# cmaestre/pcl_tracking

Hardware: AMD Instinct MI355X
Metric: particles x input-points / sec per frame (tracked frames/sec @8192 particles per GPU) (higher is better)
Workload: dtype f32

## Files before the change

include/pft.h:

```cpp
#ifndef PFT_H
#define PFT_H

#include <stddef.h>
#include <stdint.h>

#ifdef __cplusplus
extern "C" {
#endif

#define PFT_ABI_VERSION 5

typedef struct pft_point_xyzrgba {
  float x, y, z, w;
  uint32_t rgba;
  uint32_t pad[3];
} pft_point_xyzrgba;

typedef struct pft_particle {
  float x, y, z, w;
  float roll, pitch, yaw, weight;
} pft_particle;

typedef enum pft_status {
  PFT_OK = 0,
// ... 143 lines not shown
  int32_t min_pairs;
  double pair_distance;
  double inlier_distance;
  double margin;
  double trans_eps, rot_eps;
  int32_t apply;
} pft_refine_config;

typedef struct pft_refine_score {
  uint32_t n_pairs, n_inliers;
  double sum_sq_dist, inlier_sq_dist;
} pft_refine_score;

typedef struct pft_refine_result {
  uint32_t status, iterations, n_reference, n_crop;
  double bbox[6];
  float start[12], transform[12];
  pft_particle pose;
  pft_refine_score before, after;
  uint32_t improved, applied;
} pft_refine_result;

typedef struct pft_refine_trace_entry {
  float transform[12];
  uint32_t n_pairs, n_inliers;
  double sums[PFT_REFINE_N_SUMS];
  double step_t2, step_r2;
} pft_refine_trace_entry;

void pft_refine_config_default(pft_refine_config* cfg);
int pft_refine(pft_tracker* t, const float* start12, const pft_refine_config* cfg, pft_refine_result* out);
int pft_get_refine_trace(pft_tracker* t, pft_refine_trace_entry* entries, size_t cap, size_t* n);

typedef struct pft_population_stats {
  double   sum_w, sum_w2;
  double   s[6];
  double   S[21];
  double   n_eff;
  double   mean[6];
  double   cov[36];
  double   rpy_sigma[3];
  float    pos_sigma[3];
  float    pos_axes[9];
  float    w_max;
  uint32_t n, n_zero, i_max, solve_info;
  uint32_t evaluated, uncertain, streak, flagged, calls;
} pft_population_stats;

int pft_set_spread_threshold(pft_tracker* t, double max_pos_sigma, double min_n_eff, int after);
int pft_get_spread_threshold(pft_tracker* t, double* max_pos_sigma, double* min_n_eff, int* after);
int pft_spread(pft_tracker* t);
int pft_get_spread(pft_tracker* t, pft_population_stats* out);

int pft_dist_bind(pft_tracker* t, void* bbox6_dev, void* shard_dev, void* gathered_dev);
int pft_dist_begin_frame(pft_tracker* t);
int pft_dist_phase_a(pft_tracker* t, int iteration);
int pft_dist_phase_b(pft_tracker* t);
int pft_dist_phase_c(pft_tracker* t);

int pft_set_particles(pft_tracker* t, const pft_particle* p, size_t n);
int pft_eval_weights(pft_tracker* t, const pft_particle* particles, size_t P, float* raw_w, int32_t* nn_idx,
                     float* nn_d2);
int pft_debug_get_bbox(pft_tracker* t, float bbox[6]);
int pft_debug_get_crop(pft_tracker* t, int32_t* idx, size_t cap, size_t* n);
int pft_debug_get_input_records(pft_tracker* t, void* out, size_t first, size_t n);
int pft_debug_get_octree(pft_tracker* t, int32_t* depth, double min_xyz[3], double max_xyz[3], uint32_t* n_leaves,
                         uint32_t* n_nodes);
int pft_debug_get_point_keys(pft_tracker* t, uint32_t* keys3, size_t cap_points);
int pft_debug_get_scan_stats(pft_tracker* t, uint64_t* queries, uint64_t* scanned_points);
#define PFT_TREE_INFO_WORDS 64
int pft_debug_get_tree(pft_tracker* t, uint32_t* info, uint32_t* words, size_t words_cap, uint32_t* leaf_order,
                       size_t leaf_order_cap, void* leaf_pts, size_t leaf_pts_cap, void* crop_pts, size_t crop_pts_cap,
                       uint16_t* jump, size_t jump_cap);
int pft_debug_set_limits(pft_tracker* t, uint32_t max_words, int sorted_npass);
int pft_debug_state_save(pft_tracker* t);
int pft_debug_state_restore(pft_tracker* t);
int pft_debug_inject_error(pft_tracker* t, uint32_t bits);
int pft_debug_get_host_stat(pft_tracker* t, uint32_t out4[4]);
int pft_debug_get_ticks(pft_tracker* t, uint64_t* ticks32);
int pft_debug_get_descent_stats(pft_tracker* t, uint64_t* dbg32);
int pft_debug_get_hard_steps(pft_tracker* t, uint64_t out5[5]);
int pft_debug_get_likelihood_layout(pft_tracker* t, uint32_t out4[4]);
int pft_debug_get_ancestor_table(pft_tracker* t, uint32_t info10[10], uint32_t* table, size_t cap);
int pft_debug_aabb_support_subset(const pft_point_xyzrgba* pts, size_t n, uint32_t* keep, size_t* n_keep);
#ifdef PFT_DIAG
void pft_debug_set_ablate(pft_tracker* t, int mask);
#endif
int pft_debug_likelihood_occupancy(void);
int pft_debug_normalize(pft_tracker* t, float* w_inout, size_t n, double* fit_ratio);
int pft_debug_alias(pft_tracker* t, const float* w, size_t n, int32_t* a, double* q);
int pft_debug_weighted_mean(pft_tracker* t, const pft_particle* p, size_t n, pft_particle* out);
int pft_debug_init_particles(pft_tracker* t, const pft_particle* rep, uint32_t id_offset, size_t n_local,
                             pft_particle* out);
int pft_debug_resample(pft_tracker* t, const pft_particle* old, size_t n_total, const int32_t* a, const double* q,
                       const pft_particle* rep, uint32_t epoch, uint32_t id_offset, size_t n_local,
                       pft_particle* out);
int pft_debug_resample_prefix(pft_tracker* t, const pft_particle* old, size_t n_total, const pft_particle* rep,
                              uint32_t epoch, uint32_t id_offset, size_t n_local, int instance, pft_particle* out,
                              float* mats12);
int pft_debug_pose_to_matrix(pft_tracker* t, const pft_particle* p, size_t n, float* m12);
int pft_debug_kld_resample(pft_tracker* t, const pft_particle* old, size_t n_old, const int32_t* a, const double* q,
                           const pft_particle* motion, uint32_t epoch, pft_particle* out, int32_t* bins6,
                           uint32_t* n_out, uint32_t* k_out);
double pft_kld_normal_quantile(double u);
double pft_kld_bound(int k, double delta, double epsilon);

enum {
  PFT_K_RESAMPLE = 0, PFT_K_AABB = 1, PFT_K_CROP = 2, PFT_K_OCTREE = 3, PFT_K_LIKELIHOOD = 4,
  PFT_K_POPULATION = 5, PFT_K_PACK = 6, PFT_K_COUNT = 7
};
int pft_profile_enable(pft_tracker* t, int on);
int pft_profile_get(pft_tracker* t, int kernel_id, double* total_ms, uint64_t* launches);
int pft_profile_reset(pft_tracker* t);
const char* pft_kernel_name(int kernel_id);

#ifdef __cplusplus
}
#endif
#endif
```

pcl_tracking_amd/_lib.py:

```python
import ctypes as C
import os

_HERE = os.path.dirname(os.path.abspath(__file__))
LIB_PATH = os.environ.get("PFT_LIB_PATH") or os.path.join(_HERE, "_build", "libpft_hip.so")

PFT_ABI_VERSION = 5
PFT_SUM_TREE, PFT_SUM_PCL = 0, 1
PFT_CD_RING = 32
PFT_TREE_INFO_WORDS = 64
K_RESAMPLE, K_AABB, K_CROP, K_OCTREE, K_LIKELIHOOD, K_POPULATION, K_PACK, K_COUNT = range(8)

STATUS = {0: "ok", 1: "invalid argument", 2: "no input cloud", 3: "no reference cloud", 4: "no usable HIP device",
          5: "HIP error", 6: "capacity exceeded", 7: "invalid state", 8: "object not recognized"}


class PftError(RuntimeError):
    def __init__(self, status, detail=""):
        self.status = status
        super().__init__("pft status %d (%s) %s" % (status, STATUS.get(status, "?"), detail))


class Config(C.Structure):
    _fields_ = [
        ("abi_version", C.c_uint32), ("device_id", C.c_int32), ("stream", C.c_void_p),
# ... 97 lines not shown
        ("abi_version", C.c_uint32), ("device_id", C.c_int32), ("stream", C.c_void_p),
        ("stream_is_external", C.c_int32),
        ("pass_enable", C.c_int32), ("pass_field", C.c_int32), ("pass_min", C.c_float), ("pass_max", C.c_float),
        ("pass_negative", C.c_int32),
        ("voxel_mode", C.c_int32), ("leaf_size", C.c_float * 3), ("approx_hist_size", C.c_uint32),
        ("max_points", C.c_uint32),
    ]


VOXEL_NONE, VOXEL_APPROX, VOXEL_EXACT = 0, 1, 2


class SegmentConfig(C.Structure):
    _fields_ = [
        ("abi_version", C.c_uint32), ("device_id", C.c_int32), ("stream", C.c_void_p),
        ("stream_is_external", C.c_int32),
        ("transform_enable", C.c_int32), ("transform", C.c_float * 16),
        ("plane_enable", C.c_int32), ("max_iterations", C.c_int32), ("distance_threshold", C.c_double),
        ("probability", C.c_double), ("seed", C.c_uint32), ("optimize_coefficients", C.c_int32),
        ("box_enable", C.c_int32 * 3), ("box_min", C.c_float * 3), ("box_max", C.c_float * 3),
        ("cluster_tolerance", C.c_double), ("min_cluster_size", C.c_int32), ("max_cluster_size", C.c_int32),
        ("max_points", C.c_uint32),
    ]


class SegmentPlane(C.Structure):
    _fields_ = [
        ("status", C.c_int32), ("n_valid", C.c_uint32), ("coefficients", C.c_float * 4),
        ("ransac_coefficients", C.c_float * 4), ("sample", C.c_int32 * 3), ("ransac_inliers", C.c_uint32),
        ("inliers", C.c_uint32), ("iterations", C.c_uint32), ("hypotheses_scored", C.c_uint32),
        ("n_survivors", C.c_uint32),
    ]


PLANE_FOUND, PLANE_NONE, PLANE_DISABLED = 0, 1, 2
SEGMENT_MAX_PLANES = 16
ROUNDS_STOP_FRACTION, ROUNDS_STOP_NO_PLANE, ROUNDS_STOP_MAX_PLANES = 0, 1, 2
SEGMENT_STAGES = ("compaction", "sample", "score", "replay", "refit", "cluster", "output")
MODEL_STAGES = ("remove_zero_points", "centroid", "recentre", "grid_sample")

_vp, _sz, _i32, _u32, _u64, _f64 = C.c_void_p, C.c_size_t, C.c_int32, C.c_uint32, C.c_uint64, C.c_double
_P = C.POINTER
SYMBOLS = [
    ("pft_config_default", None, [_P(Config)]),
    ("pft_status_string", C.c_char_p, [C.c_int]),
    ("pft_create", C.c_int, [_P(Config), _P(_vp)]),
    ("pft_destroy", None, [_vp]),
    ("pft_last_error_string", C.c_char_p, [_vp]),
    ("pft_set_reference", C.c_int, [_vp, _vp, _sz]),
    ("pft_set_trans", C.c_int, [_vp, _vp]),
    ("pft_set_input", C.c_int, [_vp, _vp, _sz]),
    ("pft_set_input_device", C.c_int, [_vp, _vp, _sz]),
    ("pft_set_input_from_filter", C.c_int, [_vp, _vp, _sz]),
    ("pft_compute", C.c_int, [_vp]),
    ("pft_get_result", C.c_int, [_vp, _vp]),
    ("pft_get_particles", C.c_int, [_vp, _vp, _sz, _P(_sz)]),
    ("pft_to_matrix", None, [_vp, _vp]),
    ("pft_to_state", None, [_vp, _vp]),
    ("pft_get_fit_ratio", C.c_int, [_vp, _P(_f64)]),
    ("pft_synchronize", C.c_int, [_vp]),
    ("pft_dist_bind", C.c_int, [_vp, _vp, _vp, _vp]),
    ("pft_dist_begin_frame", C.c_int, [_vp]),
    ("pft_dist_phase_a", C.c_int, [_vp, C.c_int]),
    ("pft_dist_phase_b", C.c_int, [_vp]),
    ("pft_dist_phase_c", C.c_int, [_vp]),
    ("pft_set_particles", C.c_int, [_vp, _vp, _sz]),
    ("pft_eval_weights", C.c_int, [_vp, _vp, _sz, _vp, _vp, _vp]),
    ("pft_debug_get_bbox", C.c_int, [_vp, _vp]),
    ("pft_debug_get_crop", C.c_int, [_vp, _vp, _sz, _P(_sz)]),
    ("pft_debug_get_input_records", C.c_int, [_vp, _vp, _sz, _sz]),
    ("pft_debug_get_octree", C.c_int, [_vp, _P(_i32), _vp, _vp, _P(_u32), _P(_u32)]),
    ("pft_debug_get_point_keys", C.c_int, [_vp, _vp, _sz]),
    ("pft_debug_get_tree", C.c_int, [_vp, _vp, _vp, _sz, _vp, _sz, _vp, _sz, _vp, _sz, _vp, _sz]),
    ("pft_debug_get_scan_stats", C.c_int, [_vp, _P(_u64), _P(_u64)]),
    ("pft_debug_set_limits", C.c_int, [_vp, _u32, C.c_int]),
    ("pft_debug_inject_error", C.c_int, [_vp, _u32]),
    ("pft_debug_state_save", C.c_int, [_vp]),
    ("pft_debug_state_restore", C.c_int, [_vp]),
    ("pft_debug_get_host_stat", C.c_int, [_vp, _vp]),
    ("pft_debug_get_ticks", C.c_int, [_vp, _vp]),
    ("pft_debug_get_descent_stats", C.c_int, [_vp, _vp]),
    ("pft_debug_get_likelihood_layout", C.c_int, [_vp, _vp]),
    ("pft_debug_get_ancestor_table", C.c_int, [_vp, _vp, _vp, _sz]),
    ("pft_debug_get_hard_steps", C.c_int, [_vp, _vp]),
    ("pft_debug_aabb_support_subset", C.c_int, [_vp, C.c_size_t, _vp, _vp]),
    ("pft_debug_likelihood_occupancy", C.c_int, []),
    ("pft_debug_normalize", C.c_int, [_vp, _vp, _sz, _P(_f64)]),
    ("pft_debug_alias", C.c_int, [_vp, _vp, _sz, _vp, _vp]),
    ("pft_debug_weighted_mean", C.c_int, [_vp, _vp, _sz, _vp]),
    ("pft_debug_init_particles", C.c_int, [_vp, _vp, _u32, _sz, _vp]),
    ("pft_debug_resample", C.c_int, [_vp, _vp, _sz, _vp, _vp, _vp, _u32, _u32, _sz, _vp]),
    ("pft_debug_resample_prefix", C.c_int, [_vp, _vp, _sz, _vp, _u32, _u32, _sz, C.c_int, _vp, _vp]),
    ("pft_debug_pose_to_matrix", C.c_int, [_vp, _vp, _sz, _vp]),
    ("pft_debug_kld_resample", C.c_int, [_vp, _vp, _sz, _vp, _vp, _vp, _u32, _vp, _vp, _P(_u32), _P(_u32)]),
    ("pft_set_change_detector", C.c_int, [_vp, C.c_int, C.c_int, C.c_int, _f64]),
    ("pft_get_change_detector", C.c_int, [_vp, _P(C.c_int), _P(C.c_int), _P(C.c_int), _P(_f64)]),
    ("pft_debug_change_state", C.c_int, [_vp, C.c_int, _P(_u32), _P(_u32), _vp, _P(_i32), _vp, _P(_u32)]),
    ("pft_debug_change_detect", C.c_int, [_vp, _vp, _sz, C.c_int, _f64, C.c_int, _vp, _sz, _P(_sz)]),
    ("pft_set_report_cloud", C.c_int, [_vp, _vp, _sz]),
    ("pft_report", C.c_int, [_vp]),
    ("pft_get_report", C.c_int, [_vp, _P(ObjectReport)]),
    ("pft_get_tracked_cloud", C.c_int, [_vp, _vp, _sz, _P(_sz)]),
    ("pft_set_match_threshold", C.c_int, [_vp, _f64, C.c_int]),
    ("pft_get_match_threshold", C.c_int, [_vp, _P(_f64), _P(C.c_int)]),
    ("pft_match", C.c_int, [_vp]),
    ("pft_get_match", C.c_int, [_vp, _P(MatchStatsStruct)]),
    ("pft_get_match_pairs", C.c_int, [_vp, _vp, _vp, _sz, _P(_sz)]),
    ("pft_reset_tracking", C.c_int, [_vp]),
    ("pft_set_spread_threshold", C.c_int, [_vp, _f64, _f64, C.c_int]),
    ("pft_get_spread_threshold", C.c_int, [_vp, _P(_f64), _P(_f64), _P(C.c_int)]),
    ("pft_spread", C.c_int, [_vp]),
    ("pft_get_spread", C.c_int, [_vp, _P(PopulationStatsStruct)]),
    ("pft_reacquire_config_default", None, [_P(ReacquireConfig)]),
    ("pft_reacquire", C.c_int, [_vp, _vp, _sz, _P(ReacquireConfig), _P(ReacquireResultStruct)]),
    ("pft_reacquire_from_segmenter", C.c_int, [_vp, _vp, _P(ReacquireConfig), _P(ReacquireResultStruct)]),
    ("pft_get_reacquire_scores", C.c_int, [_vp, _vp, _vp, _vp, _vp, _vp, _vp, _vp, _vp, _sz, _P(_sz)]),
    ("pft_refine_config_default", None, [_P(RefineConfig)]),
    ("pft_refine", C.c_int, [_vp, _vp, _P(RefineConfig), _P(RefineResultStruct)]),
    ("pft_get_refine_trace", C.c_int, [_vp, _vp, _sz, _P(_sz)]),
    ("pft_kld_normal_quantile", _f64, [_f64]),
    ("pft_kld_bound", _f64, [C.c_int, _f64, _f64]),
    ("pft_profile_enable", C.c_int, [_vp, C.c_int]),
    ("pft_profile_get", C.c_int, [_vp, C.c_int, _P(_f64), _P(_u64)]),
    ("pft_profile_reset", C.c_int, [_vp]),
    ("pft_kernel_name", C.c_char_p, [C.c_int]),
    ("pft_filter_default_config", None, [_P(FilterConfig)]),
    ("pft_filter_create", C.c_int, [_P(FilterConfig), _P(_vp)]),
    ("pft_filter_destroy", None, [_vp]),
    ("pft_filter_last_error_string", C.c_char_p, [_vp]),
    ("pft_filter_apply", C.c_int, [_vp, _vp, _sz]),
    ("pft_filter_apply_device", C.c_int, [_vp, _vp, _sz]),
    ("pft_filter_apply_async", C.c_int, [_vp, _vp, _sz]),
    ("pft_filter_apply_device_async", C.c_int, [_vp, _vp, _sz]),
    ("pft_filter_counts", C.c_int, [_vp, _P(_sz), _P(_sz)]),
    ("pft_filter_output_device", C.c_int, [_vp, _P(_vp), _P(_sz)]),
    ("pft_filter_get_output", C.c_int, [_vp, _vp, _sz, _P(_sz)]),
    ("pft_filter_get_pass_indices", C.c_int, [_vp, _vp, _sz, _P(_sz)]),
    ("pft_filter_last_ms", C.c_int, [_vp, _P(_f64)]),
    ("pft_segment_default_config", None, [_P(SegmentConfig)]),
    ("pft_segment_create", C.c_int, [_P(SegmentConfig), _P(_vp)]),
    ("pft_segment_destroy", None, [_vp]),
    ("pft_segment_last_error_string", C.c_char_p, [_vp]),
    ("pft_segment_apply", C.c_int, [_vp, _vp, _sz]),
    ("pft_segment_apply_device", C.c_int, [_vp, _vp, _sz]),
    ("pft_segment_get_plane", C.c_int, [_vp, _P(SegmentPlane)]),
    ("pft_segment_get_plane_inliers", C.c_int, [_vp, C.c_int, _vp, _sz, _P(_sz)]),
    ("pft_segment_cluster_count", C.c_int, [_vp, _P(_sz)]),
    ("pft_segment_cluster_sizes", C.c_int, [_vp, _vp, _sz]),
    ("pft_segment_get_cluster_indices", C.c_int, [_vp, _vp, _sz, _P(_sz)]),
    ("pft_segment_get_cluster_points", C.c_int, [_vp, _vp, _sz, _P(_sz)]),
    ("pft_segment_last_ms", C.c_int, [_vp, _P(_f64), _vp]),
    ("pft_debug_segment_hypotheses", C.c_int, [_vp, _vp, _vp, _sz, _P(_sz)]),
    ("pft_segment_set_plane_rounds", C.c_int, [_vp, C.c_int, _f64]),
    ("pft_segment_get_plane_rounds", C.c_int, [_vp, _P(C.c_int), _P(_f64)]),
    ("pft_segment_plane_count", C.c_int, [_vp, _P(_sz), _P(C.c_int)]),
    ("pft_segment_get_plane_round", C.c_int, [_vp, _sz, _P(SegmentPlane)]),
    ("pft_segment_get_plane_round_inliers", C.c_int, [_vp, _sz, C.c_int, _vp, _sz, _P(_sz)]),
    ("pft_segment_set_refit_order", C.c_int, [_vp, C.c_int]),
    ("pft_debug_segment_round_hypotheses", C.c_int, [_vp, _sz, _vp, _vp, _sz, _P(_sz)]),
    ("pft_segment_clusters_device", C.c_int, [_vp, _P(_vp), _P(_sz)]),
    ("pft_model_create", C.c_int, [C.c_int, _P(_vp)]),
    ("pft_model_destroy", None, [_vp]),
    ("pft_model_last_error_string", C.c_char_p, [_vp]),
    ("pft_model_prepare", C.c_int, [_vp, _vp, _sz, C.c_float]),
    ("pft_model_prepare_device", C.c_int, [_vp, _vp, _sz, C.c_float]),
    ("pft_model_prepare_from_segment", C.c_int, [_vp, _vp, _sz, C.c_float]),
# ... 58 lines not shown
```

pcl_tracking_amd/csrc/pft_api.hip:

```cpp
#include <math.h>
#include <stdio.h>
#include <string.h>

#include <stdlib.h>

#include <algorithm>
#include <cmath>
#include <string>
#include <vector>

#include "pft_internal.h"
#include "../../include/pft_segment.h"

#define HIPCHK(t, call)                                                                       \
  do {                                                                                        \
    hipError_t e_ = (call);                                                                   \
    if (e_ != hipSuccess) {                                                                   \
      (t)->err = std::string(#call) + ": " + hipGetErrorString(e_);                           \
      return PFT_ERR_HIP;                                                                     \
    }                                                                                         \
  } while (0)

struct EvPair {
  hipEvent_t a, b;
// ... 72 lines not shown
  PftHeader* d_hdr = nullptr;
  int32_t* d_nn_idx = nullptr;
  float* d_nn_d2 = nullptr;
  size_t nn_cap = 0;
  pft_particle* d_dbg_part = nullptr;
  size_t dbg_part_cap = 0;
  PftHeader* d_dbg_hdr = nullptr;
  float* d_dbg_f = nullptr;
  size_t dbg_f_cap = 0;
  void *bound_bbox6 = nullptr, *bound_shard = nullptr, *bound_gathered = nullptr;

  pft_particle* sv_part = nullptr;
  int32_t* sv_alias_list = nullptr;
  double* sv_alias_pref = nullptr;
  uint32_t* sv_alias_pos = nullptr;
  PftHeader* sv_hdr = nullptr;
  int sv_cur = 0;
  uint32_t sv_epoch = 0;
  bool sv_changed = false, sv_valid = false;

  int cd_use = 0;
  uint32_t cd_interval = 10, cd_min_points = 10;
  double cd_res = 0.01, cd_res_latched = 0.01;
  bool cd_latched = false, cd_ever = false, gate_on = false;
  uint32_t cd_counter = 0;
  CdInst cd, cd_dbg;
  double cd_dbg_res = 0.01;
  PftChangeState* sv_cd = nullptr;
  unsigned long long* sv_cd_key[2] = {nullptr, nullptr};
  uint32_t* sv_cd_cnt[2] = {nullptr, nullptr};
  uint32_t sv_cd_cap = 0;
  bool sv_cd_valid = false;
  uint32_t sv_cd_counter = 0;

  pft_point_xyzrgba* d_rep_pts = nullptr;
  pft_point_xyzrgba* d_rep_tracked = nullptr;
  pft_object_report* d_report = nullptr;
  uint32_t rep_n = 0, rep_cap = 0;
  uint32_t rep_tracked_n = 0;
  bool rep_issued = false;

  pft_match_stats* d_match = nullptr;
  int32_t* d_match_idx = nullptr;
  float* d_match_d2 = nullptr;
  uint32_t match_cap = 0;
  uint32_t match_n = 0;
  bool match_issued = false;
  bool tree_of_compute = false;
  double match_min_ratio = 0.0;
  int match_lost_after = 1;

  pft_population_stats* d_spread = nullptr;
  double* d_spread_part = nullptr;
  uint32_t *d_spread_zero = nullptr, *d_spread_imax = nullptr;
  float* d_spread_wmax = nullptr;
  bool spread_issued = false;
  double spread_max_pos_sigma = INFINITY, spread_min_n_eff = 0.0;
  int spread_after = 1;

  pft_particle* d_rq_part = nullptr;
  float* d_rq_mats = nullptr;
  PftRqScores rq_sc = {};
  uint32_t rq_cap = 0;
  float* d_rq_centres = nullptr;
  uint32_t *d_rq_first = nullptr, *d_rq_count = nullptr;
  uint32_t rq_centres_cap = 0;
  float* d_rq_bbox_part = nullptr;
  pft_reacquire_result* d_rq_result = nullptr;
  uint32_t rq_n = 0;
  bool rq_valid = false;
  std::vector<float> rq_centres;
  PftRefineDev rf = {};
  float* d_rf_mats = nullptr;
  uint32_t rf_n = 0;
  bool rf_valid = false;

  bool has_ref = false, has_input = false, initialized = false, changed = false;
  uint32_t resample_epoch = 0;
  float trans[16];

  bool use_graph = false;
  hipGraphExec_t graph_exec = nullptr;
  uint32_t graph_frames = 0, graph_rebuilds = 0;

  bool prof = false;
  std::vector<EvPair> ev[PFT_K_COUNT];
  std::vector<EvPair> ev_free;
  double prof_ms[PFT_K_COUNT] = {0};
  uint64_t prof_n[PFT_K_COUNT] = {0};
};

static const char* k_names[PFT_K_COUNT] = {"resample", "aabb", "crop", "octree", "likelihood", "population", "pack"};

extern "C" const char* pft_kernel_name(int id) { return (id >= 0 && id < PFT_K_COUNT) ? k_names[id] : "?"; }

extern "C" const char* pft_status_string(int s) {
  switch (s) {
    case PFT_OK: return "ok";
    case PFT_ERR_INVALID_ARG: return "invalid argument";
    case PFT_ERR_NO_INPUT: return "no input cloud";
    case PFT_ERR_NO_REFERENCE: return "no reference cloud";
    case PFT_ERR_NO_DEVICE: return "no usable HIP device (there is no CPU fallback)";
    case PFT_ERR_HIP: return "HIP error";
    case PFT_ERR_CAPACITY: return "capacity exceeded";
    case PFT_ERR_STATE: return "invalid state";
    case PFT_ERR_LOST: return "object not recognized";
  }
  return "unknown";
}

extern "C" void pft_config_default(pft_config* c) {
  memset(c, 0, sizeof(*c));
  c->abi_version = PFT_ABI_VERSION;
  c->device_id = 0;
  c->stream = nullptr;
  c->stream_is_external = 0;
  c->particle_num = 400;
  c->iteration_num = 2;
  for (int k = 0; k < 6; k++) {
    c->step_noise_cov[k] = 0.015 * 0.015;
    c->initial_noise_cov[k] = 0.00001;
    c->initial_noise_mean[k] = 0.0;
  }
  c->step_noise_cov[3] *= 40.0;
  c->step_noise_cov[4] *= 40.0;
  c->step_noise_cov[5] *= 40.0;
  c->alpha = 15.0;
  c->resample_likelihood_thr = 0.0;
  c->max_distance = 0.1;
  c->octree_resolution = 0.01;
  c->distance_weight = 1.0;
  c->hsv_weight = 0.1;
  c->h_weight = 1.0;
  c->s_weight = 1.0;
  c->v_weight = 0.0;
  c->hsv_pcl180_argorder = 1;
  c->use_normal = 0;
  c->seed = 1;
  c->rank = 0;
  c->world_size = 1;
  c->kld_adaptive = 0;
  c->maximum_particle_num = 500;
  c->kld_delta = 0.99;
  c->kld_epsilon = 0.2;
  for (int k = 0; k < 6; k++) c->kld_bin_size[k] = 0.1;
  c->motion_ratio = 0.25;
  c->exact_nearest = 0;
  c->sum_order = PFT_SUM_TREE;
}

extern "C" double pft_kld_normal_quantile(double u) {
  static const double a[9] = {1.24818987e-4, -1.075204047e-3, 5.198775019e-3, -0.019198292004, 0.059054035642,
                              -0.151968751364, 0.319152932694, -0.5319230073, 0.797884560593};
  static const double b[15] = {-4.5255659e-5, 1.5252929e-4, -1.9538132e-5, -6.76904986e-4, 1.390604284e-3,
                               -7.9462082e-4, -2.034254874e-3, 6.549791214e-3, -0.010557625006, 0.011630447319,
                               -9.279453341e-3, 5.353579108e-3, -2.141268741e-3, 5.35310849e-4, 9.99936657524e-1};
  double w, y, z;
  if (u == 0.) return 0.5;
  y = u / 2.0;
  if (y < -6.) return 0.0;
  if (y > 6.) return 1.0;
  if (y < 0.) y = -y;
  if (y < 1.) {
    w = y * y;
    z = a[0];
    for (int i = 1; i < 9; i++) z = z * w + a[i];
// ... 221 lines not shown
  dfree(t->sort.keys[0]); dfree(t->sort.keys[1]); dfree(t->sort.vals[0]); dfree(t->sort.vals[1]);
  dfree(t->sort.hist); dfree(t->sort.tile_cnt); dfree(t->sort.tile_box);
  uint32_t cap = n;
  t->max_words = cap * 8u + 64u;
  HIPCHK(t, dalloc(&t->d_in_raw, cap));
  HIPCHK(t, dalloc(&t->d_in_pts, cap));
  HIPCHK(t, dalloc(&t->d_crop_counts, (size_t)(cap / 1024 + 2)));
  HIPCHK(t, dalloc(&t->d_crop_slots, (size_t)(cap / 1024 + 2)));
  HIPCHK(t, hipMemsetAsync(t->d_crop_slots, 0, (size_t)(cap / 1024 + 2) * sizeof(unsigned long long), t->stream));
  HIPCHK(t, dalloc(&t->d_crop_pts, cap));
  HIPCHK(t, dalloc(&t->d_crop_idx, cap));
  HIPCHK(t, dalloc(&t->d_words, t->max_words));
  HIPCHK(t, dalloc(&t->d_leaf_pts, cap));
  HIPCHK(t, dalloc(&t->d_leaf_order, cap));
  HIPCHK(t, dalloc(&t->d_pt_node, cap));
  HIPCHK(t, dalloc(&t->d_pt_key, (size_t)cap * 3));
  HIPCHK(t, dalloc(&t->d_pt_tmp, cap));
  HIPCHK(t, dalloc(&t->d_pt_key64, cap));
  t->sort.ntiles = (cap + 1023u) / 1024u;
  HIPCHK(t, dalloc(&t->sort.keys[0], cap));
  HIPCHK(t, dalloc(&t->sort.keys[1], cap));
  HIPCHK(t, dalloc(&t->sort.vals[0], cap));
  HIPCHK(t, dalloc(&t->sort.vals[1], cap));
  HIPCHK(t, dalloc(&t->sort.hist, (size_t)256 * t->sort.ntiles + 256));
  HIPCHK(t, dalloc(&t->sort.tile_cnt, (size_t)t->sort.ntiles * (PFT_MAX_DEPTH + 2)));
  HIPCHK(t, dalloc(&t->sort.tile_box, (size_t)t->sort.ntiles * 6));
  t->in_cap = cap;
  return PFT_OK;
}

static void cd_free(CdInst& c) {
  dfree(c.b.st); dfree(c.b.set_key[0]); dfree(c.b.set_key[1]); dfree(c.b.set_cnt[0]); dfree(c.b.set_cnt[1]);
  dfree(c.b.tab_key); dfree(c.b.tab_cnt); dfree(c.b.pt_key); dfree(c.b.mark); dfree(c.pts);
  c.b.cap = c.b.tab_cap = 0;
}
static int cd_reserve(pft_tracker* t, CdInst& c, uint32_t cap, bool debug) {
  if (cap < 1024u) cap = 1024u;
  if (c.b.st && cap <= c.b.cap) return PFT_OK;
  CdInst n;
  uint32_t tab = 64u;
  while (tab < 4u * cap) tab <<= 1;
  HIPCHK(t, dalloc(&n.b.st, 1));
  for (int k = 0; k < 2; k++) {
    HIPCHK(t, dalloc(&n.b.set_key[k], cap));
    HIPCHK(t, dalloc(&n.b.set_cnt[k], cap));
  }
  HIPCHK(t, dalloc(&n.b.tab_key, tab));
  HIPCHK(t, dalloc(&n.b.tab_cnt, tab));
  HIPCHK(t, dalloc(&n.b.pt_key, cap));
  if (debug) {
    HIPCHK(t, dalloc(&n.b.mark, cap));
    HIPCHK(t, dalloc(&n.pts, cap));
  }
  n.b.cap = cap;
  n.b.tab_cap = tab;
  if (c.b.st) {
    HIPCHK(t, hipMemcpyAsync(n.b.st, c.b.st, sizeof(PftChangeState), hipMemcpyDeviceToDevice, t->stream));
    for (int k = 0; k < 2; k++) {
      HIPCHK(t, hipMemcpyAsync(n.b.set_key[k], c.b.set_key[k], (size_t)c.b.cap * 8u, hipMemcpyDeviceToDevice, t->stream));
      HIPCHK(t, hipMemcpyAsync(n.b.set_cnt[k], c.b.set_cnt[k], (size_t)c.b.cap * 4u, hipMemcpyDeviceToDevice, t->stream));
    }
    HIPCHK(t, hipStreamSynchronize(t->stream));
  } else {
    HIPCHK(t, hipMemsetAsync(n.b.st, 0, sizeof(PftChangeState), t->stream));
  }
  cd_free(c);
  c = n;
  return PFT_OK;
}

PftSwitches pft_read_switches() {
  auto on = [](const char* name) { return getenv(name) != nullptr; };
  auto is1 = [](const char* name) { const char* e = getenv(name); return e && e[0] == '1'; };
  PftSwitches w = {};
  w.graph = is1("PFT_GRAPH");
  if (const char* b = getenv("PFT_FORCE_BUILDER")) w.builder = !strcmp(b, "single") ? 1 : (!strcmp(b, "sorted") ? 2 : 0);
  w.leaf_indirect = on("PFT_LEAF_INDIRECT") ? (int)is1("PFT_LEAF_INDIRECT") : -1;
  w.aabb_full = on("PFT_AABB_FULL");
  w.resample_one_lane = on("PFT_RESAMPLE_ONE_LANE");
  w.split_resample = on("PFT_SPLIT_RESAMPLE") || w.resample_one_lane;
  w.crop_two_pass = on("PFT_CROP_TWO_PASS");
  w.generic_descent = is1("PFT_GENERIC_DESCENT");
  w.ancestor_table = !on("PFT_ANCESTOR_TABLE") || is1("PFT_ANCESTOR_TABLE");
  w.exact_path = on("PFT_EXACT_SHELLS_ONLY") ? PftExactPath::shells : on("PFT_EXACT_PER_QUERY") ? PftExactPath::per_query : PftExactPath::sorted;
#ifdef PFT_DIAG
  if (const char* a = getenv("PFT_ABLATE")) w.ablate = atoi(a);
  w.skip_octree = on("PFT_DEBUG_SKIP_OCTREE");
#endif
  return w;
}

#ifdef PFT_DIAG
extern "C" void pft_debug_set_ablate(pft_tracker* t, int mask) { if (t) t->sw.ablate = mask; }
#endif

extern "C" int pft_create(const pft_config* cfg, pft_tracker** out) {
  if (!cfg || !out) return PFT_ERR_INVALID_ARG;
  *out = nullptr;
  if (cfg->abi_version != PFT_ABI_VERSION || cfg->particle_num <= 0 || cfg->iteration_num <= 0 ||
      cfg->world_size <= 0 || cfg->rank < 0 || cfg->rank >= cfg->world_size || cfg->use_normal != 0 ||
      cfg->particle_num % cfg->world_size != 0 || !(cfg->octree_resolution > 0) ||
      (cfg->sum_order != PFT_SUM_TREE && cfg->sum_order != PFT_SUM_PCL))
    return PFT_ERR_INVALID_ARG;
  if (cfg->particle_num > PFT_MAX_PARTICLES) return PFT_ERR_CAPACITY;
  if (cfg->kld_adaptive) {
    if (cfg->world_size != 1 || cfg->maximum_particle_num <= 0 || !(cfg->kld_epsilon > 0)) return PFT_ERR_INVALID_ARG;
    for (int k = 0; k < 6; k++)
      if (!(cfg->kld_bin_size[k] > 0)) return PFT_ERR_INVALID_ARG;
    if (cfg->maximum_particle_num >= PFT_POPM_MIN || cfg->particle_num >= PFT_POPM_MIN) return PFT_ERR_CAPACITY;
  }
  int ndev = 0;
  if (hipGetDeviceCount(&ndev) != hipSuccess || ndev <= 0 || cfg->device_id >= ndev) return PFT_ERR_NO_DEVICE;
  if (hipSetDevice(cfg->device_id) != hipSuccess) return PFT_ERR_NO_DEVICE;
  hipDeviceProp_t prop;
  if (hipGetDeviceProperties(&prop, cfg->device_id) != hipSuccess) return PFT_ERR_NO_DEVICE;

  pft_tracker* t = new pft_tracker();
  t->cfg = *cfg;
  t->num_cus = prop.multiProcessorCount > 0 ? prop.multiProcessorCount : 256;
  if (cfg->stream_is_external) {
    t->stream = static_cast<hipStream_t>(cfg->stream);
  } else {
    if (hipStreamCreateWithFlags(&t->stream, hipStreamNonBlocking) != hipSuccess) {
      delete t;
      return PFT_ERR_HIP;
    }
    t->own_stream = true;
  }
  for (int i = 0; i < 16; i++) t->trans[i] = (i % 5 == 0) ? 1.0f : 0.0f;
  t->sw = pft_read_switches();
  t->use_graph = t->sw.graph && t->own_stream;

  PftParams& p = t->prm;
  memset(&p, 0, sizeof(p));
  p.alpha = cfg->alpha;
  p.maxd2 = cfg->max_distance * cfg->max_distance;
  p.res = cfg->octree_resolution;
  p.dist_w = cfg->distance_weight;
  p.hsv_w = cfg->hsv_weight;
  p.h_w = (float)cfg->h_weight;
  p.s_w = (float)cfg->s_weight;
  p.v_w = (float)cfg->v_weight;
  p.hsv_argorder = cfg->hsv_pcl180_argorder;
  for (int k = 0; k < 6; k++) {
    p.step_sigma[k] = sqrt(cfg->step_noise_cov[k]);
    p.init_sigma[k] = sqrt(cfg->initial_noise_cov[k]);
    p.init_mean[k] = cfg->initial_noise_mean[k];
  }
  p.seed_lo = (uint32_t)cfg->seed;
  p.seed_hi = (uint32_t)(cfg->seed >> 32);
  p.P_total = (uint32_t)cfg->particle_num;
  p.P_local = p.P_total / (uint32_t)cfg->world_size;
  p.id_offset = p.P_local * (uint32_t)cfg->rank;
  p.M = 0;
  p.nchunk = 1;
  p.ref_chunk = PFT_REF_CHUNK;
  p.split_last = 0;
  p.kld = cfg->kld_adaptive ? 1u : 0u;
  p.kld_max = (uint32_t)cfg->maximum_particle_num;
  p.kld_z = pft_kld_normal_quantile(cfg->kld_delta);
  p.kld_eps = cfg->kld_epsilon;
  for (int k = 0; k < 6; k++) p.kld_bin[k] = (float)cfg->kld_bin_size[k];
  p.motion_ratio = cfg->motion_ratio;
  p.sum_order = cfg->sum_order;
  t->Pcap = p.kld && p.kld_max > p.P_total ? p.kld_max : p.P_total;

// ... 290 lines not shown
  }
  if (!t->d_n_in) {
    HIPCHK(t, dalloc(&t->d_n_in, 1));
    HIPCHK(t, hipMemsetAsync(t->d_n_in, 0, sizeof(uint32_t), t->stream));
  }
  if (!t->borrow || !t->borrow->filter_alive || t->borrow_of != f) {
    release_borrow(t);
    PftBorrow* b = new PftBorrow();
    if (hipEventCreateWithFlags(&b->ev, hipEventDisableTiming) != hipSuccess) {
      delete b;
      t->err = "pft_set_input_from_filter: hipEventCreateWithFlags failed";
      return PFT_ERR_HIP;
    }
    t->borrow = b;
    t->borrow_of = f;
    pftf_attach(f, b);
  }
  t->borrow->armed = true;
  t->borrow->valid = true;
  HIPCHK(t, hipStreamWaitEvent(t->stream, v.done, 0));
  t->N = (uint32_t)bound;
  t->n_on_device = true;
  t->n_src = v.n_out_dev;
  t->raw_pending = v.out;
  t->has_input = true;
  sync_dev(t);
  return PFT_OK;
}

static void stage_init_particles(pft_tracker* t) {
  pft_particle rep;
  pft_to_state(t->trans, &rep);
  rep.weight = 1.0f / (float)t->prm.P_total;
  sync_dev(t);
  ProfScope ps(t, PFT_K_RESAMPLE);
  pftk_init_particles(t->stream, t->prm, rep, t->d_part[t->cur], t->d_mats, t->d_hdr);
  t->initialized = true;
  t->changed = false;
  t->resample_epoch = 0;
}

static void stage_resample(pft_tracker* t) {
  sync_dev(t);
  pft_particle* out = t->d_part[1 - t->cur];
  {
    ProfScope ps(t, PFT_K_RESAMPLE);
    if (t->prm.kld)
      pftk_resample_kld(t->stream, t->prm, t->dev, t->resample_epoch, out, nullptr, nullptr, nullptr);
    else
      pftk_resample(t->stream, t->prm, t->dev, t->resample_epoch, out, t->sw.resample_one_lane);
  }
  t->resample_epoch++;
  t->cur = 1 - t->cur;
  sync_dev(t);
}

static void stage_aabb(pft_tracker* t, const PftDev& d, uint32_t np, bool finalize) {
  ProfScope ps(t, PFT_K_AABB);
  pftk_aabb(t->stream, t->prm, d, np, finalize);
}
static void stage_resample_aabb(pft_tracker* t, bool finalize) {
  if (!t->prm.kld && t->changed && !t->sw.split_resample) {
    sync_dev(t);
    uint32_t nparts;
    {
      ProfScope ps(t, PFT_K_RESAMPLE);
      nparts = pftk_resample_box(t->stream, t->prm, t->dev, t->resample_epoch, t->d_part[1 - t->cur]);
    }
    if (nparts) {
      t->resample_epoch++;
      t->cur = 1 - t->cur;
      sync_dev(t);
      t->dev.bbox_grid = nparts;
      if (finalize) pftk_bbox_final(t->stream, t->dev);
      return;
    }
  }
  if (t->changed) stage_resample(t);
  sync_dev(t);
  stage_aabb(t, t->dev, t->prm.kld ? t->Pcap : t->prm.P_local, finalize);
}
__global__ void k_inject_error(PftHeader* hdr, uint32_t bits) { hdr->error |= bits; }

static void stage_crop_octree_likelihood(pft_tracker* t, const PftDev& d, uint32_t np, bool debug_nn,
                                         bool bbox_from_partials, bool keep_point_keys = false,
                                         bool likelihood = true) {
  {
    ProfScope ps(t, PFT_K_CROP);
    if (++t->crop_epoch == 0) t->crop_epoch = 1;
    const bool from_filter = t->n_on_device && t->raw_pending;
    pftk_crop(t->stream, t->prm, d, bbox_from_partials, t->crop_epoch, t->raw_pending, t->sw.crop_two_pass,
              from_filter ? t->n_src : nullptr);
    t->raw_pending = nullptr;
    if (from_filter && t->borrow) {
      hipEventRecord(t->borrow->ev, t->stream);
      t->borrow->recorded = true;
      t->borrow->armed = false;
    }
    if (t->inject_error & ~16u) {
      hipLaunchKernelGGL(k_inject_error, dim3(1), dim3(1), 0, t->stream, t->d_hdr, t->inject_error & ~16u);
      t->inject_error &= 16u;
    }
    if (t->gate_on) {
      PftChangeArgs a;
      a.res = t->cd_res_latched;
      a.use = t->cd_use ? 1u : 0u;
      a.interval = t->cd_interval;
      a.min_points = t->cd_min_points;
      a.force = 0u;
      pftk_change_detect(t->stream, t->cd.b, t->d_crop_pts, &t->d_hdr->n_crop, 0u, a, t->h_stat);
    }
  }
  if (t->cfg.exact_nearest) {
    PftDev dq = d;
    {
      const unsigned long long nq = (unsigned long long)np * t->prm.M;
      if (nq > t->eq_cap && nq <= (1ull << 30)) {
        dfree(t->d_eq_sorted); dfree(t->d_eq_out); dfree(t->d_eq_blk); dfree(t->d_eq_tiles);
        t->eq_cap = t->eq_blk_cap = t->eq_tiles_cap = 0;
        const size_t nblk = (size_t)(nq / 64u) + PFT_EC_SLOTS + 64u;
        size_t ppw = ((size_t)np + (size_t)t->num_cus - 1u) / (size_t)t->num_cus;
        ppw = ppw < 1u ? 1u : (ppw > 32u ? 32u : ppw);
        const size_t ntiles = ((size_t)np + ppw - 1u) / ppw + 1u;
        if (dalloc(&t->d_eq_sorted, (size_t)nq) == hipSuccess && dalloc(&t->d_eq_out, (size_t)nq) == hipSuccess &&
            dalloc(&t->d_eq_blk, nblk) == hipSuccess) {
          t->eq_cap = (uint32_t)nq;
          t->eq_blk_cap = (uint32_t)nblk;
          const size_t want = ntiles < 4096u ? ntiles : 4096u;
          if (dalloc(&t->d_eq_tiles, want * 2u * 8192u) == hipSuccess) t->eq_tiles_cap = (uint32_t)want;
          else (void)hipGetLastError();
        } else {
          (void)hipGetLastError();
          dfree(t->d_eq_sorted); dfree(t->d_eq_out); dfree(t->d_eq_blk);
        }
      }
      {
        const volatile uint32_t* hs = t->h_stat;
        const uint32_t demand = hs ? hs[4] : 0u;
        if (demand > t->ec_pool_cap && t->ec_pool_cap < PFT_EC_POOL) {
          unsigned long long want = (unsigned long long)demand + demand / 4u;
          uint32_t cap = t->ec_pool_cap;
          while (cap < want && cap < PFT_EC_POOL) cap <<= 1;
          hipStreamSynchronize(t->stream);
          float4* grown = nullptr;
          if (dalloc(&grown, (size_t)cap) == hipSuccess) {
            dfree(t->d_ec_list);
            t->d_ec_list = grown;
            t->ec_pool_cap = cap;
          } else {
            (void)hipGetLastError();
          }
        }
        dq.ec_list = t->d_ec_list;
        dq.ec_pool_cap = t->ec_pool_cap;
        t->dev.ec_list = t->d_ec_list;
        t->dev.ec_pool_cap = t->ec_pool_cap;
      }
      dq.eq_sorted = t->d_eq_sorted;
      dq.eq_out = t->d_eq_out;
      dq.eq_blk = t->d_eq_blk;
      dq.eq_cap = t->eq_cap;
      dq.eq_blk_cap = t->eq_blk_cap;
      dq.eq_tiles = t->d_eq_tiles;
      dq.eq_tiles_cap = t->eq_tiles_cap;
    }
    {
      ProfScope ps(t, PFT_K_OCTREE);
      pftk_exact_grid(t->stream, t->prm, dq);
    }
    ProfScope ps(t, PFT_K_LIKELIHOOD);
    pftk_likelihood_exact(t->stream, t->prm, dq, np, debug_nn, t->num_cus, t->sw.exact_path);
    return;
  }
  {
    ProfScope ps(t, PFT_K_OCTREE);
    PftDev db = d;
    if (!keep_point_keys) db.pt_key = nullptr;
    const volatile uint32_t* hs = t->h_stat;
    const uint32_t last_n = hs ? hs[0] : 0u, last_depth = hs ? hs[1] : 0u;
    bool sorted = last_n > PFT_SORTED_BUILD_MIN;
    if (t->sw.builder == 1) sorted = false;
    if (t->sw.builder == 2) sorted = true;
#ifdef PFT_DIAG
    if (t->sw.skip_octree && ++t->dbg_builds > 8) {
    } else
#endif
    if (sorted) {
      int npass = last_depth > 0u ? (int)((3u * (last_depth + 1u) + 7u) / 8u) : 8;
      if (t->force_npass > 0) npass = t->force_npass;
      if (npass > 8) npass = 8;
      pftk_octree_sorted(t->stream, t->prm, db, t->sort, d.N, npass);
      t->leaf_indirect = false;
    } else {
      t->leaf_indirect = t->sw.leaf_indirect >= 0 ? t->sw.leaf_indirect == 1 : (unsigned long long)np * t->prm.M <= 8000000ull;
      pftk_octree(t->stream, t->prm, db, last_n, t->leaf_indirect);
    }
  }
  if (!likelihood) return;
  {
    ProfScope ps(t, PFT_K_LIKELIHOOD);
    const int flags = (t->sw.generic_descent ? 0 : 1) | (t->sw.ancestor_table ? 2 : 0) | (t->sw.ablate << 8);
    pftk_likelihood(t->stream, t->prm, d, np, debug_nn, t->num_cus, t->leaf_indirect, flags);
  }
}

static int check_ready(pft_tracker* t) {
  if (!t) return PFT_ERR_INVALID_ARG;
  hipSetDevice(t->cfg.device_id);
  if (!t->has_input || t->N == 0) return PFT_ERR_NO_INPUT;
  if (t->n_on_device && t->raw_pending && !(t->borrow && t->borrow->valid)) {
    t->err = "the filter handed over by pft_set_input_from_filter was applied again or destroyed before the frame's first crop";
    t->has_input = false;
    t->raw_pending = nullptr;
    return PFT_ERR_NO_INPUT;
  }
  if (!t->has_ref) return PFT_ERR_NO_REFERENCE;
  return PFT_OK;
}

extern "C" int pft_compute(pft_tracker* t) {
  int r = check_ready(t);
  if (r != PFT_OK) return r;
  if (t->cfg.world_size != 1) {
    t->err = "pft_compute on a sharded handle: drive the pft_dist_* phases instead";
    return PFT_ERR_STATE;
  }
  t->tree_of_compute = false;
  if (!t->initialized) stage_init_particles(t);
  if (!t->cd_latched) {
    t->cd_res_latched = t->cd_res;
    t->cd_latched = true;
  }
  t->gate_on = t->cd_ever;
  sync_dev(t);
  auto run_iterations = [&]() {
    for (int it = 0; it < t->cfg.iteration_num; it++) {
      stage_resample_aabb(t, false);
      const uint32_t np = t->prm.kld ? t->Pcap : t->prm.P_local;
      stage_crop_octree_likelihood(t, t->dev, np, false, true);
      if (t->inject_error & 16u) {
        hipLaunchKernelGGL(k_inject_error, dim3(1), dim3(1), 0, t->stream, t->d_hdr, 16u);
        t->inject_error &= ~16u;
      }
      {
        ProfScope ps(t, PFT_K_POPULATION);
        pftk_population(t->stream, t->prm, t->dev, t->prm.kld ? t->Pcap : t->prm.P_total, 1, 1, 1, 1);
      }
      t->changed = true;
      if (!t->cd_ever) t->cd_counter = t->cd_counter == 0u ? t->cd_interval : t->cd_counter - 1u;
    }
  };
  const bool graphed = t->use_graph && !t->cfg.exact_nearest && t->changed && !t->prof && !t->n_on_device &&
                       t->graph_frames++ >= 2u;
  if (!graphed) {
    run_iterations();
  } else {
    const int cur0 = t->cur;
    const uint32_t epoch0 = t->resample_epoch, crop0 = t->crop_epoch, grid0 = t->dev.bbox_grid;
    const pft_point_xyzrgba* raw0 = t->raw_pending;
    const uint32_t cdc0 = t->cd_counter;
    hipError_t ge = hipStreamBeginCapture(t->stream, hipStreamCaptureModeThreadLocal);
    hipGraph_t g = nullptr;
    if (ge == hipSuccess) {
      run_iterations();
      ge = hipStreamEndCapture(t->stream, &g);
    }
    if (ge == hipSuccess && g) {
      bool ready = false;
      if (t->graph_exec) {
        hipGraphNode_t bad = nullptr;
        hipGraphExecUpdateResult res;
        ready = hipGraphExecUpdate(t->graph_exec, g, &bad, &res) == hipSuccess;
        if (!ready) {
          (void)hipGetLastError();
          hipGraphExecDestroy(t->graph_exec);
          t->graph_exec = nullptr;
        }
      }
      if (!ready) {
        ge = hipGraphInstantiate(&t->graph_exec, g, nullptr, nullptr, 0);
        t->graph_rebuilds++;
        ready = ge == hipSuccess;
      }
      if (ready) ge = hipGraphLaunch(t->graph_exec, t->stream);
    } else if (ge == hipSuccess) {
      ge = hipErrorUnknown;
    }
    if (g) hipGraphDestroy(g);
    if (ge != hipSuccess) {
      (void)hipGetLastError();
      if (t->graph_exec) {
        hipGraphExecDestroy(t->graph_exec);
        t->graph_exec = nullptr;
      }
      t->use_graph = false;
      t->cur = cur0;
      t->resample_epoch = epoch0;
      t->crop_epoch = crop0;
      t->dev.bbox_grid = grid0;
      t->raw_pending = raw0;
      t->cd_counter = cdc0;
      sync_dev(t);
      run_iterations();
    }
  }
  t->gate_on = false;
  sync_dev(t);
  hipError_t e = hipGetLastError();
  if (e != hipSuccess) {
    t->err = std::string("kernel launch: ") + hipGetErrorString(e);
    return PFT_ERR_HIP;
  }
  t->tree_of_compute = true;
  return PFT_OK;
}

extern "C" int pft_dist_bind(pft_tracker* t, void* bbox6_dev, void* shard_dev, void* gathered_dev) {
  if (!t || !bbox6_dev || !shard_dev || !gathered_dev) return PFT_ERR_INVALID_ARG;
  t->bound_bbox6 = bbox6_dev;
  t->bound_shard = shard_dev;
  t->bound_gathered = gathered_dev;
  sync_dev(t);
  return PFT_OK;
}

extern "C" int pft_dist_begin_frame(pft_tracker* t) {
  int r = check_ready(t);
  if (r != PFT_OK) return r;
  if (!t->bound_gathered) {
    t->err = "pft_dist_bind not called";
    return PFT_ERR_STATE;
  }
  if (!t->initialized) stage_init_particles(t);
  return PFT_OK;
}

extern "C" int pft_dist_phase_a(pft_tracker* t, int iteration) {
  (void)iteration;
  int r = check_ready(t);
  if (r != PFT_OK) return r;
  if (!t->initialized) return PFT_ERR_STATE;
  stage_resample_aabb(t, true);
  return PFT_OK;
}

extern "C" int pft_dist_phase_b(pft_tracker* t) {
  int r = check_ready(t);
  if (r != PFT_OK) return r;
  sync_dev(t);
  stage_crop_octree_likelihood(t, t->dev, t->prm.P_local, false, false);
  {
// ... 170 lines not shown
  t->resample_epoch = t->sv_epoch;
  t->changed = t->sv_changed;
  t->cd_counter = t->sv_cd_counter;
  sync_dev(t);
  CopySegs cs;
  state_segments(t, false, &cs);
  hipLaunchKernelGGL(k_copy_segments, dim3(64, 5), dim3(256), 0, t->stream, cs);
  if (t->sv_cd_valid) {
    const uint32_t cap = t->sv_cd_cap;
    HIPCHK(t, hipMemcpyAsync(t->cd.b.st, t->sv_cd, sizeof(PftChangeState), hipMemcpyDeviceToDevice, t->stream));
    for (int k = 0; k < 2; k++) {
      HIPCHK(t, hipMemcpyAsync(t->cd.b.set_key[k], t->sv_cd_key[k], (size_t)cap * 8u, hipMemcpyDeviceToDevice, t->stream));
      HIPCHK(t, hipMemcpyAsync(t->cd.b.set_cnt[k], t->sv_cd_cnt[k], (size_t)cap * 4u, hipMemcpyDeviceToDevice, t->stream));
    }
  }
  return PFT_OK;
}

extern "C" int pft_debug_inject_error(pft_tracker* t, uint32_t bits) {
  if (!t) return PFT_ERR_INVALID_ARG;
  t->inject_error = bits;
  return PFT_OK;
}
extern "C" int pft_debug_get_host_stat(pft_tracker* t, uint32_t out4[4]) {
  if (!t || !out4 || !t->h_stat) return PFT_ERR_INVALID_ARG;
  for (int i = 0; i < 4; i++) out4[i] = ((volatile uint32_t*)t->h_stat)[i];
  return PFT_OK;
}
static int ensure_dbg_part(pft_tracker* t, size_t n) {
  if (n > t->dbg_part_cap) {
    hipStreamSynchronize(t->stream);
    dfree(t->d_dbg_part);
    HIPCHK(t, dalloc(&t->d_dbg_part, n));
    t->dbg_part_cap = n;
  }
  return PFT_OK;
}
static int ensure_dbg_f(pft_tracker* t, size_t n) {
  if (n > t->dbg_f_cap) {
    hipStreamSynchronize(t->stream);
    dfree(t->d_dbg_f);
    HIPCHK(t, dalloc(&t->d_dbg_f, n));
    t->dbg_f_cap = n;
  }
  return PFT_OK;
}

extern "C" int pft_eval_weights(pft_tracker* t, const pft_particle* particles, size_t P, float* raw_w,
                                int32_t* nn_idx, float* nn_d2) {
  int r = check_ready(t);
  if (r != PFT_OK) return r;
  if (!particles || !P) return PFT_ERR_INVALID_ARG;
  if (P > (t->prm.kld ? t->Pcap : t->prm.P_local)) {
    t->err = "pft_eval_weights: " + std::to_string(P) + " particles handed over, the handle's buffers hold " +
             std::to_string(t->prm.kld ? t->Pcap : t->prm.P_local) + " (particle_num / maximum_particle_num of this rank)";
    return PFT_ERR_CAPACITY;
  }
  r = ensure_dbg_part(t, P);
  if (r != PFT_OK) return r;
  r = ensure_dbg_f(t, P);
  if (r != PFT_OK) return r;
  const bool want_nn = nn_idx || nn_d2;
  const size_t pairs = P * (size_t)t->prm.M;
  if (want_nn && pairs > t->nn_cap) {
    hipStreamSynchronize(t->stream);
    dfree(t->d_nn_idx);
    dfree(t->d_nn_d2);
    HIPCHK(t, dalloc(&t->d_nn_idx, pairs));
    HIPCHK(t, dalloc(&t->d_nn_d2, pairs));
    t->nn_cap = pairs;
  }
  sync_dev(t);
  t->tree_of_compute = false;
  PftDev d = t->dev;
  d.p_active = nullptr;
  d.part_cur = t->d_dbg_part;
  d.part_all = t->d_dbg_part;
  d.bbox6 = t->d_bbox6;
  HIPCHK(t, hipMemcpyAsync(t->d_dbg_part, particles, P * sizeof(pft_particle), hipMemcpyHostToDevice, t->stream));
  HIPCHK(t, hipMemsetAsync(&t->d_hdr->stat_queries, 0, (2 + 32) * sizeof(unsigned long long), t->stream));
  HIPCHK(t, hipMemsetAsync(t->d_hdr->dbg_hard, 0, sizeof(t->d_hdr->dbg_hard) + sizeof(t->d_hdr->lik_layout), t->stream));
  pftk_pose_to_matrix(t->stream, t->d_dbg_part, (uint32_t)P, t->d_mats);
  stage_aabb(t, d, (uint32_t)P, false);
  stage_crop_octree_likelihood(t, d, (uint32_t)P, want_nn, true, true);
  pftk_finalize_raw(t->stream, t->prm, d, (uint32_t)P, t->d_dbg_f, nullptr);
  if (raw_w) HIPCHK(t, hipMemcpyAsync(raw_w, t->d_dbg_f, P * sizeof(float), hipMemcpyDeviceToHost, t->stream));
  if (nn_idx) HIPCHK(t, hipMemcpyAsync(nn_idx, t->d_nn_idx, pairs * sizeof(int32_t), hipMemcpyDeviceToHost, t->stream));
  if (nn_d2) HIPCHK(t, hipMemcpyAsync(nn_d2, t->d_nn_d2, pairs * sizeof(float), hipMemcpyDeviceToHost, t->stream));
  HIPCHK(t, hipStreamSynchronize(t->stream));
  if (t->initialized) pftk_pose_to_matrix(t->stream, t->d_part[t->cur], t->prm.P_local, t->d_mats);
  HIPCHK(t, hipGetLastError());
  return check_device_error(t);
}

static int read_hdr(pft_tracker* t, PftHeader* h) {
  HIPCHK(t, hipMemcpyAsync(h, t->d_hdr, sizeof(PftHeader), hipMemcpyDeviceToHost, t->stream));
  HIPCHK(t, hipStreamSynchronize(t->stream));
  return PFT_OK;
}

extern "C" int pft_debug_get_bbox(pft_tracker* t, float bbox[6]) {
  if (!t || !bbox) return PFT_ERR_INVALID_ARG;
  PftHeader h;
  int r = read_hdr(t, &h);
  if (r != PFT_OK) return r;
  memcpy(bbox, h.bbox, sizeof(float) * 6);
  return PFT_OK;
}

extern "C" int pft_debug_get_crop(pft_tracker* t, int32_t* idx, size_t cap, size_t* n) {
  if (!t) return PFT_ERR_INVALID_ARG;
  PftHeader h;
  int r = read_hdr(t, &h);
  if (r != PFT_OK) return r;
  if (n) *n = h.n_crop;
  size_t c = cap < h.n_crop ? cap : h.n_crop;
  if (idx && c) {
    HIPCHK(t, hipMemcpy(idx, t->d_crop_idx, c * sizeof(int32_t), hipMemcpyDeviceToHost));
  }
  return PFT_OK;
}

extern "C" int pft_debug_get_input_records(pft_tracker* t, void* out, size_t first, size_t n) {
  if (!t || (!out && n)) return PFT_ERR_INVALID_ARG;
  if (first + n > t->in_cap) return PFT_ERR_CAPACITY;
  hipSetDevice(t->cfg.device_id);
  HIPCHK(t, hipStreamSynchronize(t->stream));
  if (n) HIPCHK(t, hipMemcpy(out, t->d_in_pts + first, n * sizeof(float4), hipMemcpyDeviceToHost));
  return PFT_OK;
}

extern "C" int pft_debug_get_octree(pft_tracker* t, int32_t* depth, double mn[3], double mx[3], uint32_t* n_leaves,
                                    uint32_t* n_nodes) {
  if (!t) return PFT_ERR_INVALID_ARG;
  PftHeader h;
  int r = read_hdr(t, &h);
  if (r != PFT_OK) return r;
  if (h.error) {
    t->err = "octree build error flag " + std::to_string(h.error);
    return PFT_ERR_CAPACITY;
  }
  if (depth) *depth = h.depth;
  if (mn) memcpy(mn, h.omin, sizeof(double) * 3);
  if (mx) memcpy(mx, h.omax, sizeof(double) * 3);
  if (n_leaves) *n_leaves = h.n_leaves;
  if (n_nodes) *n_nodes = h.n_words;
  return PFT_OK;
}

extern "C" int pft_debug_get_point_keys(pft_tracker* t, uint32_t* keys3, size_t cap_points) {
  if (!t || !keys3) return PFT_ERR_INVALID_ARG;
  PftHeader h;
  int r = read_hdr(t, &h);
  if (r != PFT_OK) return r;
  size_t c = cap_points < h.n_crop ? cap_points : h.n_crop;
  if (c) HIPCHK(t, hipMemcpy(keys3, t->d_pt_key, c * 3 * sizeof(uint32_t), hipMemcpyDeviceToHost));
  return PFT_OK;
}

extern "C" int pft_debug_get_tree(pft_tracker* t, uint32_t* info, uint32_t* words, size_t words_cap, uint32_t* leaf_order,
                                  size_t leaf_order_cap, void* leaf_pts, size_t leaf_pts_cap, void* crop_pts,
                                  size_t crop_pts_cap, uint16_t* jump, size_t jump_cap) {
  if (!t || !info) return PFT_ERR_INVALID_ARG;
  if (t->cfg.world_size != 1 || t->cfg.exact_nearest) {
    t->err = "pft_debug_get_tree: sharded handles (world_size > 1) and the exact nearest-neighbour mode build no octree";
    return PFT_ERR_INVALID_ARG;
  }
  if (t->in_cap == 0 || !t->d_words) {
    t->err = "pft_debug_get_tree before the first input cloud: no tree buffers yet";
    return PFT_ERR_STATE;
  }
  hipSetDevice(t->cfg.device_id);
  PftHeader h;
  int r = read_hdr(t, &h);
  if (r != PFT_OK) return r;
  const size_t n_jump = (size_t)1 << (3 * PFT_JUMP_MAX_LEVEL);
  uint32_t f32[5];
  memcpy(&f32[0], &h.margin_cells, 4);
  memcpy(&f32[1], &h.inv_res, 4);
  memcpy(&f32[2], h.ominf, 12);
  memset(info, 0, PFT_TREE_INFO_WORDS * sizeof(uint32_t));
  info[0] = h.n_crop; info[1] = h.error; info[2] = (uint32_t)h.depth; info[3] = (uint32_t)h.use_table;
  info[4] = h.n_words; info[5] = h.n_leaves; info[6] = h.leaf_start; info[7] = (uint32_t)h.n_grow;
  info[8] = (uint32_t)h.build_path; info[9] = (uint32_t)h.leaf_indirect; info[10] = (uint32_t)h.jump_level;
  for (int k = 0; k < 5; k++) info[11 + k] = f32[k];
  info[16] = h.build_epoch; info[17] = h.build_variant;
  info[18] = ((uint32_t)pftk_max_lds_bytes() - 10240u) & ~15u;
  info[19] = (uint32_t)n_jump;
  static_assert(20 + PFT_MAX_DEPTH + 3 <= PFT_TREE_INFO_WORDS, "lvl_start does not fit the info block");
  for (int l = 0; l <= h.depth + 1 && l < PFT_MAX_DEPTH + 3 && h.depth > 0; l++) info[20 + l] = h.lvl_start[l];
  const size_t n_pts = std::min<size_t>(h.n_crop, t->in_cap);
  const size_t n_words = std::min<size_t>(h.n_words, (size_t)t->in_cap * 8u + 64u);
  auto copy = [&](void* dst, const void* src, size_t cap, size_t count, size_t elem) -> hipError_t {
    const size_t c = std::min(cap, count);
    return dst && src && c ? hipMemcpy(dst, src, c * elem, hipMemcpyDeviceToHost) : hipSuccess;
  };
  HIPCHK(t, copy(words, t->d_words, words_cap, n_words, sizeof(uint32_t)));
  HIPCHK(t, copy(leaf_order, t->d_leaf_order, leaf_order_cap, n_pts, sizeof(uint32_t)));
  HIPCHK(t, copy(leaf_pts, t->d_leaf_pts, leaf_pts_cap, n_pts, sizeof(float4)));
  HIPCHK(t, copy(crop_pts, t->d_crop_pts, crop_pts_cap, n_pts, sizeof(float4)));
  HIPCHK(t, copy(jump, t->d_jump, jump_cap, n_jump, sizeof(uint16_t)));
  return PFT_OK;
}

extern "C" int pft_debug_get_ticks(pft_tracker* t, uint64_t* ticks32) {
  if (!t || !ticks32) return PFT_ERR_INVALID_ARG;
  PftHeader h;
  int r = read_hdr(t, &h);
  if (r != PFT_OK) return r;
  for (int i = 0; i < 32; i++) ticks32[i] = h.ticks[i];
  return PFT_OK;
}

extern "C" int pft_debug_aabb_support_subset(const pft_point_xyzrgba* pts, size_t n, uint32_t* keep, size_t* n_keep) {
  if ((!pts && n) || !keep || !n_keep) return PFT_ERR_INVALID_ARG;
  std::vector<uint32_t> k;
  pft_aabb_support_subset(pts, n, k);
  for (size_t i = 0; i < k.size(); i++) keep[i] = k[i];
  *n_keep = k.size();
  return PFT_OK;
}

extern "C" int pft_debug_get_descent_stats(pft_tracker* t, uint64_t* dbg32) {
  if (!t || !dbg32) return PFT_ERR_INVALID_ARG;
  PftHeader h;
  int r = read_hdr(t, &h);
  if (r != PFT_OK) return r;
  for (int i = 0; i < 32; i++) dbg32[i] = h.dbg[i];
  dbg32[30] = t->prm.M_box;
  dbg32[31] = t->prm.M;
  if (t->cfg.exact_nearest) {
    dbg32[8] = h.ec_nslots;
    dbg32[9] = h.ec_pool_used;
    dbg32[10] = h.eq_totals & 0xffffffffull;
    dbg32[11] = h.eq_totals >> 32;
    dbg32[12] = h.eg_ncells;
    dbg32[13] = h.n_crop;
  }
  return PFT_OK;
}

extern "C" int pft_debug_get_likelihood_layout(pft_tracker* t, uint32_t out4[4]) {
  if (!t || !out4) return PFT_ERR_INVALID_ARG;
  PftHeader h;
  int r = read_hdr(t, &h);
  if (r != PFT_OK) return r;
  memcpy(out4, h.lik_layout, sizeof(h.lik_layout));
  return PFT_OK;
}

extern "C" int pft_debug_get_ancestor_table(pft_tracker* t, uint32_t info10[10], uint32_t* table, size_t cap) {
  if (!t || !info10) return PFT_ERR_INVALID_ARG;
  PftHeader h;
  int r = read_hdr(t, &h);
  if (r != PFT_OK) return r;
  const bool has = t->d_anc != nullptr && h.anc_level > 0;
  info10[0] = has && h.anc_epoch == h.build_epoch ? 1u : 0u;
  info10[1] = has ? (uint32_t)h.anc_level : 0u;
  for (int a = 0; a < 3; a++) {
    info10[2 + a] = has ? h.anc_lo[a] : 0u;
    info10[5 + a] = has ? h.anc_bits[a] : 0u;
  }
  info10[8] = h.build_epoch;
  info10[9] = h.anc_epoch;
  const size_t cells = has ? (size_t)1 << (h.anc_bits[0] + h.anc_bits[1] + h.anc_bits[2]) : 0u;
  if (table && cells && cap) {
    HIPCHK(t, hipMemcpyAsync(table, t->d_anc, std::min(cap, cells) * sizeof(uint32_t), hipMemcpyDeviceToHost, t->stream));
    HIPCHK(t, hipStreamSynchronize(t->stream));
  }
  return PFT_OK;
}

extern "C" int pft_debug_get_hard_steps(pft_tracker* t, uint64_t out5[5]) {
  if (!t || !out5) return PFT_ERR_INVALID_ARG;
  PftHeader h;
  int r = read_hdr(t, &h);
  if (r != PFT_OK) return r;
  for (int i = 0; i < 5; i++) out5[i] = h.dbg_hard[i];
  return PFT_OK;
}

extern "C" int pft_debug_get_scan_stats(pft_tracker* t, uint64_t* queries, uint64_t* scanned) {
  if (!t) return PFT_ERR_INVALID_ARG;
  PftHeader h;
  int r = read_hdr(t, &h);
  if (r != PFT_OK) return r;
  if (queries) *queries = h.stat_queries;
  if (scanned) *scanned = h.stat_scanned;
  return PFT_OK;
}

struct DbgPop {
  pft_particle* part = nullptr;
  int32_t* a = nullptr;
  double* q = nullptr;
  int32_t* list = nullptr;
  double* pref = nullptr;
  uint32_t* pos = nullptr;
  ~DbgPop() {
    dfree(part); dfree(a); dfree(q); dfree(list); dfree(pref); dfree(pos);
  }
};

static int dbg_population(pft_tracker* t, std::vector<pft_particle>& host, int norm, int mean, int alias, DbgPop& b,
                          PftHeader* hout) {
  const size_t n = host.size();
  if (n > PFT_MAX_PARTICLES) return PFT_ERR_CAPACITY;
  HIPCHK(t, dalloc(&b.part, n));
  HIPCHK(t, dalloc(&b.a, n));
  HIPCHK(t, dalloc(&b.q, n));
  HIPCHK(t, dalloc(&b.list, 2 * n));
  HIPCHK(t, dalloc(&b.pref, 2 * n));
  HIPCHK(t, dalloc(&b.pos, n));
  HIPCHK(t, hipMemcpyAsync(b.part, host.data(), n * sizeof(pft_particle), hipMemcpyHostToDevice, t->stream));
  HIPCHK(t, hipMemsetAsync(t->d_dbg_hdr, 0, sizeof(PftHeader), t->stream));
  sync_dev(t);
  PftDev d = t->dev;
  d.p_active = nullptr;
  d.part_all = b.part;
  d.alias_list = b.list;
  d.alias_pref = b.pref;
  d.alias_pos = b.pos;
  d.hdr = t->d_dbg_hdr;
  pftk_population(t->stream, t->prm, d, (uint32_t)n, 0, norm, mean, alias);
  if (alias) pftk_alias_materialize(t->stream, d, (uint32_t)n, b.a, b.q);
  HIPCHK(t, hipMemcpyAsync(host.data(), b.part, n * sizeof(pft_particle), hipMemcpyDeviceToHost, t->stream));
  if (hout) HIPCHK(t, hipMemcpyAsync(hout, t->d_dbg_hdr, sizeof(PftHeader), hipMemcpyDeviceToHost, t->stream));
  HIPCHK(t, hipStreamSynchronize(t->stream));
  HIPCHK(t, hipGetLastError());
  return PFT_OK;
// ... 983 lines not shown
```

pcl_tracking_amd/csrc/pft_device_utils.h:

```cpp
#pragma once
#include <float.h>
#include <math.h>

#include "pft_internal.h"

#define WAVE 64
#define UNROLL_FENCE(j, every) do { if (((j) % (every)) == (every) - 1) __builtin_amdgcn_sched_barrier(0); } while (0)

__device__ __forceinline__ bool pft_unchanged(const uint32_t* gate) { return gate && *gate == 0u; }

__device__ __forceinline__ int lane_id() { return threadIdx.x & (WAVE - 1); }
__device__ __forceinline__ int wave_id() { return threadIdx.x >> 6; }

template <typename T>
__device__ __forceinline__ T wave_sum(T v) {
#pragma unroll
  for (int o = 32; o > 0; o >>= 1) v += __shfl_xor(v, o);
  return v;
}
template <int CTRL, int ROW_MASK>
__device__ __forceinline__ double dpp_move_f64(double v) {
  const unsigned long long b = (unsigned long long)__double_as_longlong(v);
  const int lo = __builtin_amdgcn_update_dpp(0, (int)(uint32_t)b, CTRL, ROW_MASK, 0xf, false);
  const int hi = __builtin_amdgcn_update_dpp(0, (int)(uint32_t)(b >> 32), CTRL, ROW_MASK, 0xf, false);
// ... 110 lines not shown
      k1 += 0xBB67AE85u;
    }
    uint32_t hi0 = __umulhi(0xD2511F53u, c0), lo0 = 0xD2511F53u * c0;
    uint32_t hi1 = __umulhi(0xCD9E8D57u, c2), lo1 = 0xCD9E8D57u * c2;
    uint32_t n0 = hi1 ^ c1 ^ k0, n1 = lo1, n2 = hi0 ^ c3 ^ k1, n3 = lo0;
    c0 = n0; c1 = n1; c2 = n2; c3 = n3;
  }
  o[0] = c0; o[1] = c1; o[2] = c2; o[3] = c3;
}

__device__ __forceinline__ double u53(uint32_t a, uint32_t b) {
  unsigned long long m = ((unsigned long long)(a >> 5) << 26) | (unsigned long long)(b >> 6);
  return (double)m * (1.0 / 9007199254740992.0);
}

__device__ __forceinline__ void normal_pair(const PftParams& p, uint32_t pid, uint32_t slot, uint32_t epoch,
                                            uint32_t purpose, double& z0, double& z1) {
  uint32_t o[4];
  philox4x32(pid, slot, epoch, purpose, p.seed_lo, p.seed_hi, o);
  double u1 = 1.0 - u53(o[0], o[1]);
  double u2 = u53(o[2], o[3]);
  double r = sqrt(-2.0 * log(u1));
  double th = 6.283185307179586 * u2;
  z0 = r * cos(th);
  z1 = r * sin(th);
}

__device__ __forceinline__ void particle_sample(pft_particle& q, const PftParams& p, const double* sigma,
                                                const double* mean, uint32_t pid, uint32_t epoch, uint32_t purpose) {
  double z[6];
  normal_pair(p, pid, 1, epoch, purpose, z[0], z[1]);
  normal_pair(p, pid, 2, epoch, purpose, z[2], z[3]);
  normal_pair(p, pid, 3, epoch, purpose, z[4], z[5]);
  q.x += (float)(z[0] * sigma[0] + mean[0]);
  q.y += (float)(z[1] * sigma[1] + mean[1]);
  q.z += (float)(z[2] * sigma[2] + mean[2]);
  q.roll += (float)(z[3] * sigma[3] + mean[3]);
  q.pitch += (float)(z[4] * sigma[4] + mean[4]);
  q.yaw += (float)(z[5] * sigma[5] + mean[5]);
}

__device__ __forceinline__ float sqrt_rn_coherence(float x) {
  float s = __builtin_amdgcn_sqrtf(x);
  const float sd = __uint_as_float(__float_as_uint(s) - 1u), su = __uint_as_float(__float_as_uint(s) + 1u);
  const float ed = fmaf(-sd, s, x), eu = fmaf(-su, s, x);
  s = ed <= 0.0f ? sd : s;
  s = eu > 0.0f ? su : s;
  return s;
}

__device__ __forceinline__ void pose_to_matrix(const pft_particle& q, float* m ) {
  float A = (float)cos((double)q.yaw), B = (float)sin((double)q.yaw);
  float C = (float)cos((double)q.pitch), D = (float)sin((double)q.pitch);
  float E = (float)cos((double)q.roll), F = (float)sin((double)q.roll);
  float DE = D * E, DF = D * F;
  m[0] = A * C;  m[1] = A * DF - B * E;  m[2] = B * F + A * DE;  m[3] = q.x;
  m[4] = B * C;  m[5] = A * E + B * DF;  m[6] = B * DE - A * F;  m[7] = q.y;
  m[8] = -D;     m[9] = C * F;           m[10] = C * E;          m[11] = q.z;
}

__device__ __forceinline__ void store_matrix(float* mats, uint32_t i, const float* m) {
  float4* dst = reinterpret_cast<float4*>(mats + 12 * (size_t)i);
  dst[0] = make_float4(m[0], m[1], m[2], m[3]);
  dst[1] = make_float4(m[4], m[5], m[6], m[7]);
  dst[2] = make_float4(m[8], m[9], m[10], m[11]);
}

__device__ __forceinline__ void load_matrix(const float* mats, uint32_t i, float* T) {
  const float4* tp = reinterpret_cast<const float4*>(mats + 12 * (size_t)i);
  float4 r0 = tp[0], r1 = tp[1], r2 = tp[2];
  T[0] = r0.x; T[1] = r0.y; T[2] = r0.z; T[3] = r0.w;
  T[4] = r1.x; T[5] = r1.y; T[6] = r1.z; T[7] = r1.w;
  T[8] = r2.x; T[9] = r2.y; T[10] = r2.z; T[11] = r2.w;
}

__device__ __forceinline__ void xform(const float* T, float x, float y, float z, float& ox, float& oy, float& oz) {
  ox = T[0] * x + T[1] * y + T[2] * z + T[3];
  oy = T[4] * x + T[5] * y + T[6] * z + T[7];
  oz = T[8] * x + T[9] * y + T[10] * z + T[11];
}

#include "pft_alias.h"

__device__ inline void pft_anc_window(PftHeader* hdr, const PftDev& d, int D, bool on, const double mn[3], double res) {
  const int L = D - PFT_ANC_UP;
  on = on && d.anc != nullptr && L >= 1;
  const float inv = (float)(1.0 / res);
  uint32_t lo[3] = {0u, 0u, 0u}, bits[3] = {0u, 0u, 0u};
  for (int a = 0; a < 3 && on; a++) {
    const float om = (float)mn[a];
    const float f0 = fmaxf(floorf((hdr->bbox[2 * a] - om) * inv), 0.0f);
    const float f1 = fmaxf(floorf((hdr->bbox[2 * a + 1] - om) * inv), 0.0f);
    const uint32_t top = (1u << L) - 1u;
    const uint32_t c0 = min(f0 < 2147483648.0f ? (uint32_t)f0 >> PFT_ANC_UP : top, top);
    const uint32_t c1 = min(f1 < 2147483648.0f ? (uint32_t)f1 >> PFT_ANC_UP : top, top);
    on = c1 >= c0;
    const uint32_t n = c1 - c0 + 1u;
    bits[a] = n > 1u ? 32u - (uint32_t)__clz((int)(n - 1u)) : 0u;
    lo[a] = min(c0, (1u << L) - (1u << bits[a]));
  }
  on = on && bits[0] + bits[1] + bits[2] <= PFT_ANC_CAP_BITS;
  hdr->anc_level = on ? L : 0;
  for (int a = 0; a < 3; a++) {
    hdr->anc_lo[a] = on ? lo[a] : 0u;
    hdr->anc_bits[a] = on ? bits[a] : 0u;
  }
  hdr->build_epoch = hdr->build_epoch + 1u;
}
```

pcl_tracking_amd/csrc/pft_internal.h:

```cpp
#pragma once
#include <hip/hip_runtime.h>
#include <stdint.h>

#include <vector>

#include "../../include/pft.h"

#define PFT_MAX_DEVICES 64
#define PFT_MAX_DEPTH 30
#define PFT_TABLE_MAX_DEPTH 10
#define PFT_MAX_GROW 40
#define PFT_JUMP_MAX_LEVEL 4
#ifndef PFT_ANC_CAP_BITS
#define PFT_ANC_CAP_BITS 18
#endif
#define PFT_ANC_CAP (1u << PFT_ANC_CAP_BITS)
#ifndef PFT_ANC_UP
#define PFT_ANC_UP 2
#endif
#define PFT_REF_CHUNK 256
#ifndef PFT_BUILD_THREADS
#define PFT_BUILD_THREADS 1024
#endif
#ifndef PFT_LIK_GROUPS
#define PFT_LIK_GROUPS 64
#endif
#ifndef PFT_LIK_CTR_STRIDE
#define PFT_LIK_CTR_STRIDE 16u
#endif
#ifndef PFT_LIK_THREADS
#define PFT_LIK_THREADS 1024
#endif
#ifndef PFT_LIK_WGS_PER_CU
#define PFT_LIK_WGS_PER_CU 2
#endif
#define PFT_POP_THREADS 1024
#define PFT_SORTED_BUILD_MIN 18000
#define PFT_EG_CAP (1u << 21)
#define PFT_EC_SLOTS (1u << 19)
#define PFT_EC_POOL (1u << 24)
#define PFT_EC_POOL_MIN (1u << 20)
#define PFT_POPM_THREADS 256
#define PFT_POPM_ITEMS 16
#define PFT_POPM_MAX_WGS 256
#define PFT_POPM_MIN (16 * PFT_POP_THREADS + 1)
#define PFT_MAX_PARTICLES (PFT_POPM_MAX_WGS * PFT_POPM_THREADS * PFT_POPM_ITEMS)

struct PftParams {
  double alpha;
  double maxd2;
  double res;
  double dist_w, hsv_w;
  float h_w, s_w, v_w;
  int hsv_argorder;
  double step_sigma[6], init_sigma[6], init_mean[6];
  uint32_t seed_lo, seed_hi;
  uint32_t P_total, P_local, id_offset;
  uint32_t M, nchunk;
  uint32_t M_box;
  uint32_t ref_chunk;
  uint32_t split_last;
  uint32_t kld;
  uint32_t kld_max;
  double kld_z;
  double kld_eps;
  float kld_bin[6];
  double motion_ratio;
  int32_t sum_order;
};

struct PftHeader {
  float bbox[6];
  uint32_t n_crop;
  uint32_t error;
  double omin[3], omax[3];
  int32_t depth;
  int32_t use_table;
  uint32_t n_words;
  uint32_t n_leaves;
  uint32_t leaf_start;
  uint32_t lvl_start[PFT_MAX_DEPTH + 3];
  int32_t n_grow;
  int32_t build_path;
  uint32_t build_variant;
  int32_t leaf_indirect;
  int32_t jump_level;
  float margin_cells;
  float ominf[3];
  float inv_res;
  int32_t anc_level;
  uint32_t anc_lo[3], anc_bits[3];
  uint32_t build_epoch;
  uint32_t anc_epoch;
  uint32_t grow_idx[PFT_MAX_GROW];
  uint32_t grow_shift[PFT_MAX_GROW];
  uint32_t grow_old_depth[PFT_MAX_GROW];
  double grow_min[PFT_MAX_GROW + 1][3];
  double fit_ratio;
  pft_particle rep;
  pft_particle motion;
  uint32_t alias_m, alias_nh;
  float eg_g, eg_inv_g, eg_min[3];
  int32_t eg_dim[3];
  uint32_t eg_ncells;
  uint32_t p_active;
  uint32_t kld_k;
  unsigned long long stat_queries, stat_scanned;
  unsigned long long dbg[32];
  unsigned long long ticks[32];
  alignas(128) uint32_t lik_ctr[PFT_LIK_GROUPS * PFT_LIK_CTR_STRIDE];
  alignas(128) uint32_t ec_nslots;
  uint32_t ec_pool_used;
  unsigned long long eq_totals;
  alignas(128) uint32_t crop_ticket;
  uint32_t pop_bar[4];
  unsigned long long dbg_hard[5];
  uint32_t lik_layout[4];
};

// ... 57 lines not shown
  uint32_t eq_tiles_cap;
  uint32_t* kld_table;
  int32_t* kld_bins;
  uint32_t* host_stat;
  int32_t* nn_idx;
  float* nn_d2;
  const uint32_t* gate;
};

struct PftChangeState {
  double mn[3], mx[3];
  int32_t depth;
  uint32_t defined;
  uint32_t counter;
  uint32_t gate;
  uint32_t n_set[2];
  uint32_t prev;
  uint32_t n_calls;
  uint32_t ring[PFT_CD_RING][5];
};
struct PftChangeBufs {
  PftChangeState* st;
  unsigned long long* set_key[2];
  uint32_t* set_cnt[2];
  unsigned long long* tab_key;
  uint32_t* tab_cnt;
  unsigned long long* pt_key;
  uint32_t* mark;
  uint32_t cap, tab_cap;
};
struct PftChangeArgs {
  double res;
  uint32_t use, interval, min_points;
  uint32_t force;
};
void pftk_change_detect(hipStream_t s, const PftChangeBufs& b, const float4* pts, const uint32_t* n_ptr, uint32_t n,
                        const PftChangeArgs& a, uint32_t* host_stat);

struct PftBorrow {
  hipEvent_t ev = nullptr;
  bool recorded = false;
  bool armed = false;
  bool valid = false;
  bool tracker_alive = true, filter_alive = true;
};
struct pft_filter;
struct PftFilterView {
  const pft_point_xyzrgba* out;
  const uint32_t* n_out_dev;
  size_t n_in;
  int device_id;
  hipEvent_t done;
};
int pftf_view(pft_filter* f, PftFilterView* v);
void pftf_attach(pft_filter* f, PftBorrow* b);

void pftk_remove_zero_points(hipStream_t s, const pft_point_xyzrgba* in, uint32_t n, float4* xyz, uint8_t* flag,
                             uint32_t* tile, uint32_t* keep_idx, float4* keep_xyz, uint32_t* n_keep);
struct pft_segment;
int pftsg_device_id(const pft_segment* s);
struct pft_model;
struct PftModelView {
  const pft_point_xyzrgba* recentred;
  size_t n_recentred;
  const pft_point_xyzrgba* reference;
  size_t n_reference;
  float trans[16];
  uint32_t first_nonfinite;
  int device_id;
};
int pftm_view(const pft_model* m, PftModelView* v);

enum class PftExactPath { sorted, per_query, shells };
struct PftSwitches {
  bool graph;
  int builder;
  int leaf_indirect;
  bool aabb_full;
  bool split_resample;
  bool resample_one_lane;
  bool crop_two_pass;
  bool generic_descent;
  bool ancestor_table;
  PftExactPath exact_path;
  int ablate;
  bool skip_octree;
};
PftSwitches pft_read_switches();

void pftk_report(hipStream_t s, const pft_point_xyzrgba* pts, uint32_t n, const PftHeader* hdr, int sum_order,
                 pft_point_xyzrgba* tracked, pft_object_report* out);
void pftk_match(hipStream_t s, const PftParams& p, const PftDev& d, double min_ratio, uint32_t lost_after,
                pft_match_stats* out, int32_t* input_idx, float* sq_dist);
uint32_t pftk_spread_blocks(uint32_t n_max);
void pftk_spread(hipStream_t s, const PftDev& d, uint32_t n_max, double* part, uint32_t* part_zero, float* part_wmax,
                 uint32_t* part_imax, double max_pos_sigma, double min_n_eff, uint32_t after, pft_population_stats* out);
struct PftRqLattice {
  uint32_t n[3];
  float base[3], span[3];
};
struct PftRqScores {
  uint32_t *n_inliers, *n_matched;
  double *coherence, *sum_sq_dist, *inlier_sq_dist;
};
void pftk_reacquire_centroids(hipStream_t s, const pft_point_xyzrgba* pts, const uint32_t* first, const uint32_t* count,
                              uint32_t n_clusters, float* centres);
void pftk_reacquire_candidates(hipStream_t s, const float* centres, uint32_t K, const PftRqLattice& lat, pft_particle* part,
                               float* mats);
void pftk_reacquire_score(hipStream_t s, const PftParams& p, const PftDev& d, uint32_t K, double inlier_d2,
                          const PftRqScores& out);
void pftk_reacquire_select(hipStream_t s, const PftParams& p, const PftDev& d, const PftRqScores& sc, uint32_t K,
                           uint32_t n_centres, uint32_t per_centre, double accept_ratio, pft_reacquire_result* out);
struct PftRefineCtl;
struct PftRefineDev {
  PftRefineCtl* ctl;
  double* part;
  uint32_t* part_n;
  uint32_t g_cap;
  pft_refine_result* result;
  pft_refine_trace_entry* trace;
};
struct PftRefineArgs {
  float start[12];
  uint32_t use_rep;
  uint32_t max_iterations, min_pairs;
  double pair2, inl2, margin, trans_eps2, rot_eps2;
};
size_t pftk_refine_ctl_bytes();
uint32_t pftk_refine_blocks(uint32_t M);
void pftk_refine_init(hipStream_t s, const PftRefineArgs& a, const PftRefineDev& r, const PftHeader* hdr, float* mats);
void pftk_refine_passes(hipStream_t s, const PftParams& p, const PftDev& d, const PftRefineDev& r, const PftRefineArgs& a);
void pftk_pack_reference(hipStream_t s, const pft_point_xyzrgba* d_pts, uint32_t n, int argorder, float4* xyz,
                         float4* hsv);
void pftk_pack_input(hipStream_t s, const pft_point_xyzrgba* d_pts, uint32_t n, float4* out,
                     const uint32_t* n_dev = nullptr);
void pftk_init_particles(hipStream_t s, const PftParams& p, pft_particle rep, pft_particle* out, float* mats,
                         PftHeader* hdr);
void pftk_resample(hipStream_t s, const PftParams& p, const PftDev& d, uint32_t epoch, pft_particle* out, bool one_lane);
void pftk_bbox_final(hipStream_t s, const PftDev& d);
uint32_t pftk_resample_box(hipStream_t s, const PftParams& p, const PftDev& d, uint32_t epoch, pft_particle* out);
void pftk_resample_table(hipStream_t s, const PftParams& p, const pft_particle* old, const int32_t* a,
                         const double* q, const PftHeader* hdr, uint32_t epoch, pft_particle* out);
void pftk_pose_to_matrix(hipStream_t s, const pft_particle* p, uint32_t n, float* mats);
void pftk_aabb(hipStream_t s, const PftParams& p, const PftDev& d, uint32_t n_particles, bool finalize);
void pft_aabb_support_subset(const pft_point_xyzrgba* pts, size_t n, std::vector<uint32_t>& keep);
void pftk_exact_grid(hipStream_t s, const PftParams& p, const PftDev& d);
void pftk_likelihood_exact(hipStream_t s, const PftParams& p, const PftDev& d, uint32_t n_particles, bool debug_nn,
                           int num_cus, PftExactPath path);
void pftk_resample_kld(hipStream_t s, const PftParams& p, const PftDev& d, uint32_t epoch, pft_particle* out,
                       const int32_t* table_a, const double* table_q, int32_t* bins_out);
void pftk_crop(hipStream_t s, const PftParams& p, const PftDev& d, bool bbox_from_partials, uint32_t epoch,
               const pft_point_xyzrgba* raw, bool two_pass, const uint32_t* n_src = nullptr);
void pftk_octree(hipStream_t s, const PftParams& p, const PftDev& d, uint32_t expected_points, bool indirect);
void pftk_octree_rescue(hipStream_t s, const PftParams& p, const PftDev& d);
struct SortBufs {
  unsigned long long* keys[2];
  uint32_t* vals[2];
  uint32_t* hist;
  uint32_t* tile_cnt;
  float* tile_box;
  uint32_t ntiles;
};
void pftk_octree_sorted(hipStream_t s, const PftParams& p, const PftDev& d, const SortBufs& sb, uint32_t n_pad,
                        int npass);
void pftk_likelihood(hipStream_t s, const PftParams& p, const PftDev& d, uint32_t n_particles, bool debug_nn,
                     int num_cus, bool leaf_indirect, int flags);
void pftk_finalize_raw(hipStream_t s, const PftParams& p, const PftDev& d, uint32_t n_particles,
                       float* raw_out , pft_particle* shard );
void pftk_population(hipStream_t s, const PftParams& p, const PftDev& d, uint32_t n, int from_partials,
                     int do_normalize, int do_mean, int do_alias);
void pftk_alias_materialize(hipStream_t s, const PftDev& d, uint32_t n, int32_t* a, double* q);
int pftk_max_lds_bytes();
int pftk_cur_device();
int pftk_radix_sort_pairs(hipStream_t s, uint32_t* key[2], uint32_t* val[2], uint32_t n, int bits, uint32_t* hist);
```

pcl_tracking_amd/csrc/pft_likelihood.hip:

```cpp
#include "pft_device_utils.h"

#ifndef PFT_LIK_PENALTY
#define PFT_LIK_PENALTY 1
#endif

struct LikCtx {
  const uint32_t* words;
  const float* tab;
  uint32_t per_axis;
  const float* lut_h;
  const float* lut_s;
  const float* pen;
  const uint16_t* jump;
  int J;
  uint32_t lvlJ_start;
  const uint32_t* anc;
  uint32_t alo, abits;
  float margin, near_thr, ominx, ominy, ominz, inv_res, ncell;
  uint32_t leaf0;
  const uint16_t* leaf16;
};

struct HybridWords {
  const __attribute__((address_space(3))) uint32_t* lds;
  const uint32_t* __restrict__ glob;
  uint32_t n_lds;
  __device__ __forceinline__ uint32_t operator[](uint32_t i) const { return i < n_lds ? lds[i] : glob[i]; }
};

__device__ __forceinline__ double rcp_nr(double x) {
  double r = __builtin_amdgcn_rcp(x);
  double e = fma(-x, r, 1.0);
  r = fma(r, e, r);
  e = fma(-x, r, 1.0);
  r = fma(r, e, r);
  return r;
}

__device__ __forceinline__ bool face_violation(uint32_t kx, uint32_t ky, uint32_t kz, uint32_t lowf, uint32_t highf,
                                               int sh) {
  const uint32_t mx = (1u << sh) - 1u;
  const uint32_t rx = kx & mx, ry = ky & mx, rz = kz & mx;
  bool v = ((lowf & 1u) && rx == 0) || ((highf & 1u) && rx == mx);
  v |= ((lowf & 2u) && ry == 0) || ((highf & 2u) && ry == mx);
  v |= ((lowf & 4u) && rz == 0) || ((highf & 4u) && rz == mx);
  return v;
}

__device__ __forceinline__ int near_face_level(uint32_t k, bool low, bool high) {
  const uint32_t t = low ? k : ~k;
  const uint32_t c = min((uint32_t)(t == 0u ? -1 : __builtin_ctz(t)), 31u);
  return (low | high) ? (int)c : -1;
}

template <bool USE_TAB, bool FAST, bool DEBUG_NN, int LEAF, bool INDIRECT, typename WordPtr>
__device__ __forceinline__ void likelihood_items(const PftParams& prm, const PftDev& d, const LikCtx& cx, WordPtr W,
                                                 uint32_t n_particles, int D, uint32_t n_crop,
                                                 const double omin[3], int abl) {
  const int lane = lane_id(), w = wave_id(), nw = blockDim.x >> 6;
  const uint32_t M = prm.M, nchunk = prm.nchunk;
  const uint32_t G = min((uint32_t)PFT_LIK_GROUPS, gridDim.x), grp = blockIdx.x % G;
  const uint32_t gq = gridDim.x / G, gr = gridDim.x % G;
  const uint32_t wgs_in_grp = gq + (grp < gr ? 1u : 0u), waves_in_grp = wgs_in_grp * (uint32_t)nw;
  const uint32_t wgs_before = grp * gq + min(grp, gr);
  const uint32_t pb = (uint32_t)((unsigned long long)n_particles * wgs_before / gridDim.x);
  const uint32_t pe = (uint32_t)((unsigned long long)n_particles * (wgs_before + wgs_in_grp) / gridDim.x);
  const uint32_t np_grp = pe - pb, nbig = prm.split_last ? nchunk - prm.split_last : nchunk, nsmall = nchunk - nbig;
  const uint32_t small_len = prm.split_last ? prm.ref_chunk / prm.split_last : 0u;
  const uint32_t it_begin = 0u, it_end = np_grp * nchunk, big_items = np_grp * nbig;
  const uint32_t lw = (blockIdx.x / G) * (uint32_t)nw + (uint32_t)w;
  uint32_t* ctr = &d.hdr->lik_ctr[grp * PFT_LIK_CTR_STRIDE];
  const double res = prm.res;
  const double maxd2 = prm.maxd2;
  const double wd = prm.dist_w, whsv = prm.hsv_w;
  const float hw = prm.h_w, sw = prm.s_w, vw = prm.v_w;
  for (uint32_t item_v = it_begin + lw; item_v < it_end;) {
    const uint32_t item = (uint32_t)__builtin_amdgcn_readfirstlane((int)item_v);
    uint32_t pi, ch, cstart, clen;
    if (item < big_items) {
      pi = pb + item / nbig;
      ch = item % nbig;
      cstart = ch * prm.ref_chunk;
      clen = prm.ref_chunk;
    } else {
      const uint32_t r = item - big_items;
      pi = pb + r / nsmall;
      ch = nbig + r % nsmall;
      cstart = nbig * prm.ref_chunk + (r % nsmall) * small_len;
      clen = small_len;
    }
    float T[12];
    load_matrix(d.mats, pi, T);
    double val = 0.0;
    unsigned long long st_q = 0, st_s = 0;
    const uint32_t jend = min(M, cstart + clen);
    const uint32_t j0 = cstart + lane;
    float4 rnext = j0 < jend ? d.ref_xyz[j0] : make_float4(0, 0, 0, 0);
    for (uint32_t j = j0; j < jend; j += WAVE) {
      const float4 r = rnext;
      if (j + WAVE < jend) rnext = d.ref_xyz[j + WAVE];
      float qx, qy, qz;
      xform(T, r.x, r.y, r.z, qx, qy, qz);
      if (n_crop == 0) {
        if (DEBUG_NN) {
          const size_t o = (size_t)pi * M + d.ref_perm[j];
          d.nn_idx[o] = -1;
          d.nn_d2[o] = INFINITY;
        }
        continue;
      }
      uint32_t node = 0, jx = 1, jy = 1, jz = 1;
      int lvl = 0;
      int dbg_fast = 0, dbg_gen = 0, dbg_jump = 0, dbg_hard = 0;
      if (FAST) {
        const float tx = (qx - cx.ominx) * cx.inv_res, ty = (qy - cx.ominy) * cx.inv_res,
                    tz = (qz - cx.ominz) * cx.inv_res;
        const float flx = floorf(tx), fly = floorf(ty), flz = floorf(tz);
        const bool inside = (int)(fminf(fminf(tx, ty), tz) >= 0.0f) & (int)(fmaxf(fmaxf(tx, ty), tz) < cx.ncell);
        const float fx = tx - flx, fy = ty - fly, fz = tz - flz;
        const float mg = cx.margin, mh = 1.0f - cx.margin;
        const uint32_t kx = inside ? (uint32_t)flx : 0u, ky = inside ? (uint32_t)fly : 0u,
                       kz = inside ? (uint32_t)flz : 0u;
        int V = -1;
        const float off = fmaxf(fmaxf(fabsf(fx - 0.5f), fabsf(fy - 0.5f)), fabsf(fz - 0.5f));
        if (__builtin_amdgcn_ballot_w64(off > cx.near_thr)) {
          const int vx = near_face_level(kx, fx < mg, fx > mh), vy = near_face_level(ky, fy < mg, fy > mh),
                    vz = near_face_level(kz, fz < mg, fz > mh);
          V = max(vx, max(vy, vz));
        }
        V = inside ? V : 31;
        int lim = min(D, D - 1 - V);
        bool inw = false;
        uint32_t ae = 0u;
        if (!INDIRECT && LEAF == 1 && cx.anc) {
          const uint32_t bx = cx.abits & 0xffu, by = (cx.abits >> 8) & 0xffu, bz = cx.abits >> 16;
          const uint32_t ux = (kx >> PFT_ANC_UP) - (cx.alo & 1023u), uy = (ky >> PFT_ANC_UP) - ((cx.alo >> 10) & 1023u),
                         uz = (kz >> PFT_ANC_UP) - (cx.alo >> 20);
          inw = ((ux >> bx) | (uy >> by) | (uz >> bz)) == 0u;
          ae = cx.anc[inw ? ux | (uy << bx) | (uz << (bx + by)) : 0u];
        }
        const int a = (int)(ae >> 27);
        const bool hit = inw & (a <= lim);
        node = hit ? (ae & 0x7ffffffu) : 0u;
        lvl = hit ? a : 0;
        lim = (hit & (a < D - PFT_ANC_UP)) ? a : lim;
        if (cx.J > 0 && __builtin_amdgcn_ballot_w64(!hit)) {
          const int sh = D - cx.J;
          const uint32_t e = cx.jump[(kx >> sh) | ((ky >> sh) << cx.J) | ((kz >> sh) << (2 * cx.J))];
          const bool take = !hit & (cx.J <= lim) & (e != 0u);
          node = take ? cx.lvlJ_start + e - 1u : node;
          lvl = take ? cx.J : lvl;
          if (DEBUG_NN) dbg_jump = take ? 1 : 0;
        }
        while (lvl < lim) {
          const int sh = D - lvl - 1;
          const uint32_t c = (((kx >> sh) & 1u) << 2) | (((ky >> sh) & 1u) << 1) | ((kz >> sh) & 1u);
          const uint32_t wv = W[node];
          if (!((wv >> c) & 1u)) break;
          node = (wv >> 8) + __popc(wv & 0xffu & ((1u << c) - 1u));
          lvl++;
          dbg_fast++;
        }
        const int up = D - lvl;
        const uint32_t top = 1u << lvl;
        jx = (kx >> up) | top; jy = (ky >> up) | top; jz = (kz >> up) | top;
      }
      if ((abl & 1) && lvl < D) {
        node = cx.leaf0;
        lvl = D;
      }
      for (; lvl < D; lvl++) {
        dbg_gen++;
        const uint32_t wv = W[node];
        const uint32_t mask = wv & 0xffu, base = wv >> 8;
        float cx0, cx1, cy0, cy1, cz0, cz1;
        if (USE_TAB) {
          const float2 tx2 = *reinterpret_cast<const float2*>(cx.tab - 2 + 2u * jx);
          const float2 ty2 = *reinterpret_cast<const float2*>(cx.tab + cx.per_axis - 2 + 2u * jy);
          const float2 tz2 = *reinterpret_cast<const float2*>(cx.tab + 2u * cx.per_axis - 2 + 2u * jz);
          cx0 = tx2.x; cx1 = tx2.y; cy0 = ty2.x; cy1 = ty2.y; cz0 = tz2.x; cz1 = tz2.y;
        } else {
          const double vs = res * (double)(1u << (D - lvl - 1));
          const uint32_t pkx = jx - (1u << lvl), pky = jy - (1u << lvl), pkz = jz - (1u << lvl);
          cx0 = (float)(((double)(2u * pkx) + 0.5) * vs + omin[0]);
          cx1 = (float)(((double)(2u * pkx + 1u) + 0.5) * vs + omin[0]);
          cy0 = (float)(((double)(2u * pky) + 0.5) * vs + omin[1]);
          cy1 = (float)(((double)(2u * pky + 1u) + 0.5) * vs + omin[1]);
          cz0 = (float)(((double)(2u * pkz) + 0.5) * vs + omin[2]);
          cz1 = (float)(((double)(2u * pkz + 1u) + 0.5) * vs + omin[2]);
        }
        float dx0 = cx0 - qx, dx1 = cx1 - qx, dy0 = cy0 - qy, dy1 = cy1 - qy, dz0 = cz0 - qz, dz1 = cz1 - qz;
        float X0 = dx0 * dx0, X1 = dx1 * dx1, Y0 = dy0 * dy0, Y1 = dy1 * dy1, Z0 = dz0 * dz0, Z1 = dz1 * dz1;
        const float yz[4] = {Y0 + Z0, Y0 + Z1, Y1 + Z0, Y1 + Z1};
#if PFT_LIK_PENALTY
        const float4 pa = *reinterpret_cast<const float4*>(cx.pen + 8u * mask);
        const float4 pb = *reinterpret_cast<const float4*>(cx.pen + 8u * mask + 4u);
        const float d0 = (X0 + yz[0]) + pa.x, d1 = (X0 + yz[1]) + pa.y, d2 = (X0 + yz[2]) + pa.z, d3 = (X0 + yz[3]) + pa.w;
        const float d4 = (X1 + yz[0]) + pb.x, d5 = (X1 + yz[1]) + pb.y, d6 = (X1 + yz[2]) + pb.z, d7 = (X1 + yz[3]) + pb.w;
        float m0, m1, m2, best;
        asm("v_min3_f32 %0, %1, %2, %3" : "=v"(m0) : "v"(d0), "v"(d1), "v"(d2));
        asm("v_min3_f32 %0, %1, %2, %3" : "=v"(m1) : "v"(d3), "v"(d4), "v"(d5));
        asm("v_min3_f32 %0, %1, %2, %3" : "=v"(m2) : "v"(d6), "v"(d7), "v"(m0));
        asm("v_min_f32 %0, %1, %2" : "=v"(best) : "v"(m1), "v"(m2));
        uint32_t bc = 7u;
        bc = d6 == best ? 6u : bc;
        bc = d5 == best ? 5u : bc;
        bc = d4 == best ? 4u : bc;
        bc = d3 == best ? 3u : bc;
        bc = d2 == best ? 2u : bc;
        bc = d1 == best ? 1u : bc;
        bc = d0 == best ? 0u : bc;
#else
        float best = INFINITY;
        uint32_t bc = 0;
#pragma unroll
        for (uint32_t c = 0; c < 8; c++) {
          float dc = ((c & 4u) ? X1 : X0) + yz[c & 3u];
          bool ex = (mask >> c) & 1u;
          if (ex && dc < best) {
            best = dc;
            bc = c;
          }
        }
#endif
        if (DEBUG_NN) {
          const uint32_t ideal = ((X1 < X0) ? 4u : 0u) | ((Y1 < Y0) ? 2u : 0u) | ((Z1 < Z0) ? 1u : 0u);
          if (!((mask >> ideal) & 1u)) dbg_hard++;
        }
        node = base + __popc(mask & ((1u << bc) - 1u));
        jx = 2u * jx + ((bc >> 2) & 1u);
        jy = 2u * jy + ((bc >> 1) & 1u);
        jz = 2u * jz + (bc & 1u);
      }
      uint32_t ls, le;
// ... 47 lines not shown
        if (!(bd < INFINITY)) bpos = d.leaf_order[min(bpos, n_crop - 1u)];
      }
      const float4 bt = INDIRECT ? d.crop_pts[bpos] : d.leaf_pts[bpos];
      if (DEBUG_NN) {
        const size_t o = (size_t)pi * M + d.ref_perm[j];
        d.nn_idx[o] = INDIRECT ? (int32_t)bpos : (int32_t)d.leaf_order[bpos];
        d.nn_d2[o] = bd;
        st_q += 1;
        st_s += le - ls;
        {
          const int first = __ffsll((long long)__ballot(1)) - 1;
          const int gb = dbg_gen < 10 ? dbg_gen : 10, hb = dbg_hard < 4 ? dbg_hard : 4;
          for (int g_ = 0; g_ <= 10; g_++) {
            const unsigned long long m_ = __ballot(gb == g_);
            if (m_ && lane == first) atomicAdd(&d.hdr->dbg[g_], (unsigned long long)__popcll(m_));
          }
          for (int h_ = 0; h_ <= 4; h_++) {
            const unsigned long long m_ = __ballot(hb == h_);
            if (m_ && lane == first) atomicAdd(&d.hdr->dbg_hard[h_], (unsigned long long)__popcll(m_));
          }
          const unsigned long long mj_ = __ballot(dbg_jump != 0);
          if (mj_ && lane == first) atomicAdd(&d.hdr->dbg[11], (unsigned long long)__popcll(mj_));
        }
        int mg_ = dbg_gen, mf_ = dbg_fast, ml_ = (int)(le - ls);
        for (int o = 32; o > 0; o >>= 1) {
          mg_ = max(mg_, __shfl_xor(mg_, o));
          mf_ = max(mf_, __shfl_xor(mf_, o));
          ml_ = max(ml_, __shfl_xor(ml_, o));
        }
        if (lane == __ffsll((long long)__ballot(1)) - 1) {
          atomicAdd(&d.hdr->dbg[12], 1ull);
          atomicAdd(&d.hdr->dbg[13], (unsigned long long)mg_);
          atomicAdd(&d.hdr->dbg[14], (unsigned long long)mf_);
          atomicAdd(&d.hdr->dbg[15], (unsigned long long)ml_);
          atomicAdd(&d.hdr->dbg[16 + (mg_ < 10 ? mg_ : 10)], 1ull);
        }
      }
      if (abl & 4) {
        val += (double)bd;
      } else if ((double)bd < maxd2) {
        float ex = qx - bt.x, ey = qy - bt.y, ez = qz - bt.z;
        float n2 = (ex * ex + ey * ey) + ez * ez;
        double dist = (double)sqrt_rn_coherence(n2);
        double A = 1.0 + dist * dist * wd;
        const float4 rh = d.ref_hsv[j];
        const uint32_t pk = __float_as_uint(bt.w);
        const float th = cx.lut_h[pk & 0xffu], ts = cx.lut_s[(pk >> 8) & 0xffu], tv = cx.lut_s[(pk >> 16) & 0xffu];
        const float hd1 = fabsf(rh.x - th);
        float hd2;
        if (rh.x < th)
          hd2 = fabsf(1.0f + rh.x - th);
        else
          hd2 = fabsf(1.0f + th - rh.x);
        float h_diff;
        if (hd1 < hd2)
          h_diff = hw * hd1 * hd1;
        else
          h_diff = hw * hd2 * hd2;
        const float s_diff = sw * (rh.y - ts) * (rh.y - ts);
        const float v_diff = vw * (rh.z - tv) * (rh.z - tv);
        const float diff2 = h_diff + s_diff + v_diff;
        double Bq = 1.0 + whsv * (double)diff2;
        val += rcp_nr(A * Bq);
      }
    }
    val = wave_sum_lane63(val);
    if (lane == 63) d.partial[(size_t)pi * nchunk + ch] = val;
    {
      uint32_t nx = 0;
      if (lane == 0) nx = it_begin + waves_in_grp + atomicAdd(ctr, 1u);
      item_v = (uint32_t)__shfl((int)nx, 0);
    }
    if (DEBUG_NN) {
      st_q = wave_sum(st_q);
      st_s = wave_sum(st_s);
      if (lane == 0 && st_q) {
        atomicAdd(&d.hdr->stat_queries, st_q);
        atomicAdd(&d.hdr->stat_scanned, st_s);
      }
    }
  }
}

#define PFT_LIK_RUN(UT, FA, LF) likelihood_items<UT, FA, DEBUG_NN, LF, INDIRECT>(prm, d, cx, W, n_particles, D, n_crop, omin, abl)

template <bool DEBUG_NN, bool INDIRECT, bool GATED>
__global__ __launch_bounds__(PFT_LIK_THREADS, DEBUG_NN ? 1 : (PFT_LIK_THREADS * PFT_LIK_WGS_PER_CU) / 256) void k_likelihood(PftParams prm, PftDev d, uint32_t n_particles,
                                                                uint32_t lds_bytes, int flags) {
  const int allow_fast = flags & 1;
#ifdef PFT_DIAG
  const int abl = flags >> 8;
#else
  constexpr int abl = 0;
#endif
  extern __shared__ __attribute__((aligned(16))) unsigned char smem[];
  const PftHeader* hdr = d.hdr;
  if (GATED && pft_unchanged(d.gate)) return;
  if (d.p_active) n_particles = *d.p_active;
  const int D = hdr->depth;
  const uint32_t n_crop = (hdr->error || D <= 0 || (hdr->leaf_indirect != 0) != INDIRECT) ? 0u : hdr->n_crop;
  if (hdr->error && blockIdx.x == 0 && threadIdx.x == 0 && d.host_stat) {
    d.host_stat[2] = hdr->error;
    d.host_stat[3] |= hdr->error;
  }
  const uint32_t n_words = hdr->n_words;
  const int use_tab = hdr->use_table;
  const double omin[3] = {hdr->omin[0], hdr->omin[1], hdr->omin[2]};
  const uint32_t per_axis = use_tab ? (2u << D) : 0u;
  const bool fast = allow_fast && use_tab && hdr->margin_cells < 0.5f;
  int J = fast ? hdr->jump_level : 0;

  float* pen = reinterpret_cast<float*>(smem);
  constexpr uint32_t pen_bytes = PFT_LIK_PENALTY ? 256u * 8u * 4u : 0u;
  float* lut_h = reinterpret_cast<float*>(smem + pen_bytes);
  float* lut_s = lut_h + 256;
  float* tab = lut_s + 256;
  uint32_t used = pen_bytes + 2048u + 3u * per_axis * 4u;
  used = (used + 15u) & ~15u;
  const uint32_t leaf_start = hdr->leaf_start, n_leaves = hdr->n_leaves;
  const bool leaf16 = n_crop > 0 && n_crop < 65536u;
  const uint32_t branch_bytes = leaf16 ? leaf_start * 4u : n_words * 4u;
  const uint32_t leaf_bytes = leaf16 ? ((n_leaves + 1u) * 2u + 3u) & ~3u : 0u;
  uint32_t jump_bytes = J > 0 ? (2u << (3 * J)) : 0u;
  const bool fits_with_jump = (size_t)used + jump_bytes + branch_bytes + leaf_bytes <= (size_t)lds_bytes;
  const bool fits_without_jump = (size_t)used + branch_bytes + leaf_bytes <= (size_t)lds_bytes;
  const bool branch_only = use_tab && !fits_with_jump && leaf16 && (size_t)used + jump_bytes + branch_bytes <= (size_t)lds_bytes;
  const bool jump_dropped = !fits_with_jump && fits_without_jump && !branch_only && J > 0;
  if (!fits_with_jump && fits_without_jump && !branch_only) {
    J = 0;
    jump_bytes = 0;
  }
  uint16_t* ljump = reinterpret_cast<uint16_t*>(smem + used);
  used += jump_bytes;
  uint32_t* lwords = reinterpret_cast<uint32_t*>(smem + used);
  uint16_t* lleaf = reinterpret_cast<uint16_t*>(smem + used + branch_bytes);
  const bool words_in_lds = !branch_only && (size_t)used + branch_bytes + leaf_bytes <= (size_t)lds_bytes;
  const uint32_t n_lds_words = (words_in_lds || branch_only) ? 0u : min(n_words, (lds_bytes - used) / 4u);
  if (DEBUG_NN && blockIdx.x == 0 && threadIdx.x == 0) {
    const uint32_t layout = branch_only ? 2u : words_in_lds ? (leaf16 ? 0u : 1u) : 3u;
    const uint32_t descent = fast ? 0u : use_tab ? 1u : 2u;
    d.hdr->lik_layout[0] = 1u | (layout << 1) | (descent << 3) | (INDIRECT ? 32u : 0u) | (hdr->leaf_indirect ? 64u : 0u) |
                           (jump_dropped ? 128u : 0u) | ((uint32_t)J << 8);
    d.hdr->lik_layout[1] = n_lds_words;
    d.hdr->lik_layout[2] = lds_bytes;
    d.hdr->lik_layout[3] = __float_as_uint(hdr->margin_cells);
  }

  for (uint32_t i = threadIdx.x; i < 256; i += blockDim.x) {
    lut_h[i] = (float)i / 180.0f;
    lut_s[i] = (float)i / 255.0f;
  }
  if (PFT_LIK_PENALTY)
    for (uint32_t i = threadIdx.x; i < 2048u; i += blockDim.x) pen[i] = ((i >> 3) >> (i & 7u)) & 1u ? 0.0f : INFINITY;
  for (uint32_t e = threadIdx.x; e < 3u * per_axis; e += blockDim.x) {
    const uint32_t a = e / per_axis, r = e - a * per_axis;
    float c = 0.0f;
    if (r + 2u < per_axis) {
      const uint32_t l = 31u - (uint32_t)__clz((int)(r + 2u));
      const uint32_t k = r + 2u - (1u << l);
      const double vs = prm.res * (double)(1u << (D - (int)l));
      c = (float)(((double)k + 0.5) * vs + omin[a]);
    }
    tab[e] = c;
  }
  {
    const uint32_t* src = reinterpret_cast<const uint32_t*>(d.jump);
    uint32_t* dst = reinterpret_cast<uint32_t*>(ljump);
    for (uint32_t i = threadIdx.x; i < jump_bytes / 4u; i += blockDim.x) dst[i] = src[i];
  }
  if (words_in_lds || branch_only) {
    const uint32_t nb = leaf16 ? leaf_start : n_words;
    for (uint32_t i = threadIdx.x; i < nb; i += blockDim.x) lwords[i] = d.words[i];
    if (leaf16 && !branch_only)
      for (uint32_t i = threadIdx.x; i <= n_leaves; i += blockDim.x) lleaf[i] = (uint16_t)d.words[leaf_start + i];
  } else {
    for (uint32_t i = threadIdx.x; i < n_lds_words; i += blockDim.x) lwords[i] = d.words[i];
  }
  __syncthreads();

  LikCtx cx;
  cx.words = nullptr;
  cx.tab = tab;
  cx.per_axis = per_axis;
  cx.lut_h = lut_h;
  cx.lut_s = lut_s;
  cx.pen = pen;
  cx.jump = ljump;
  cx.J = J;
  cx.lvlJ_start = J > 0 ? hdr->lvl_start[J] : 0u;
  const bool anc_on = fast && (flags & 2) && d.anc && hdr->anc_level > 0 && hdr->anc_epoch == hdr->build_epoch;
  cx.anc = anc_on ? d.anc : nullptr;
  static_assert(PFT_TABLE_MAX_DEPTH <= 10, "ancestor table window coordinates are packed in 10 bits");
  cx.alo = hdr->anc_lo[0] | (hdr->anc_lo[1] << 10) | (hdr->anc_lo[2] << 20);
  cx.abits = hdr->anc_bits[0] | (hdr->anc_bits[1] << 8) | (hdr->anc_bits[2] << 16);
  cx.margin = hdr->margin_cells;
  cx.near_thr = 0.5f - 1.01f * hdr->margin_cells - 1.0e-6f;
  cx.ominx = hdr->ominf[0];
  cx.ominy = hdr->ominf[1];
  cx.ominz = hdr->ominf[2];
  cx.inv_res = hdr->inv_res;
  cx.ncell = (float)(1u << (D > 0 ? D : 0));
  cx.leaf0 = hdr->leaf_start;
  cx.leaf16 = lleaf;
  if (branch_only) {
    const uint32_t* W = lwords;
    if (fast)
      PFT_LIK_RUN(true, true, 2);
    else
      PFT_LIK_RUN(true, false, 2);
  } else if (words_in_lds && leaf16) {
    const uint32_t* W = lwords;
    if (fast)
      PFT_LIK_RUN(true, true, 1);
    else if (use_tab)
      PFT_LIK_RUN(true, false, 1);
    else
      PFT_LIK_RUN(false, false, 1);
  } else if (words_in_lds) {
    const uint32_t* W = lwords;
    if (fast)
      PFT_LIK_RUN(true, true, 0);
    else if (use_tab)
      PFT_LIK_RUN(true, false, 0);
    else
      PFT_LIK_RUN(false, false, 0);
  } else {
    HybridWords W;
    W.lds = (const __attribute__((address_space(3))) uint32_t*)lwords;
    W.glob = d.words;
    W.n_lds = n_lds_words;
    if (fast)
      PFT_LIK_RUN(true, true, 0);
    else if (use_tab)
      PFT_LIK_RUN(true, false, 0);
    else
      PFT_LIK_RUN(false, false, 0);
  }
}

extern "C" int pft_debug_likelihood_occupancy(void) {
  int nb = -1;
  uint32_t lds = ((uint32_t)pftk_max_lds_bytes() / (uint32_t)PFT_LIK_WGS_PER_CU) & ~255u;
  hipFuncSetAttribute(reinterpret_cast<const void*>(&k_likelihood<false, false, false>), hipFuncAttributeMaxDynamicSharedMemorySize, (int)lds);
  if (hipOccupancyMaxActiveBlocksPerMultiprocessor(&nb, reinterpret_cast<const void*>(&k_likelihood<false, false, false>), PFT_LIK_THREADS, lds) != hipSuccess) return -1;
  return nb;
}

void pftk_likelihood(hipStream_t s, const PftParams& p, const PftDev& d, uint32_t n_particles, bool debug_nn,
                     int num_cus, bool leaf_indirect, int flags) {
  static bool attr_set[PFT_MAX_DEVICES];
  uint32_t lds = ((uint32_t)pftk_max_lds_bytes() / (uint32_t)PFT_LIK_WGS_PER_CU) & ~255u;
  const int dev = pftk_cur_device();
  if (!attr_set[dev]) {
    const void* fns[8] = {
        reinterpret_cast<const void*>(&k_likelihood<false, false, false>), reinterpret_cast<const void*>(&k_likelihood<true, false, false>),
        reinterpret_cast<const void*>(&k_likelihood<false, true, false>), reinterpret_cast<const void*>(&k_likelihood<true, true, false>),
        reinterpret_cast<const void*>(&k_likelihood<false, false, true>), reinterpret_cast<const void*>(&k_likelihood<true, false, true>),
        reinterpret_cast<const void*>(&k_likelihood<false, true, true>), reinterpret_cast<const void*>(&k_likelihood<true, true, true>)};
    bool ok = true;
    for (int k = 0; k < 8; k++) ok = hipFuncSetAttribute(fns[k], hipFuncAttributeMaxDynamicSharedMemorySize, (int)lds) == hipSuccess && ok;
    attr_set[dev] = ok;
  }
  uint32_t items = n_particles * p.nchunk;
  uint32_t grid = (uint32_t)PFT_LIK_WGS_PER_CU * (uint32_t)num_cus;
  uint32_t need = (items + (PFT_LIK_THREADS / 64) - 1) / (PFT_LIK_THREADS / 64);
  if (need == 0) need = 1;
  if (grid > need) grid = need;
#define PFT_LIK_LAUNCH(DN, IND)                                                                                          \
  do {                                                                                                                   \
    if (d.gate)                                                                                                          \
      hipLaunchKernelGGL((k_likelihood<DN, IND, true>), dim3(grid), dim3(PFT_LIK_THREADS), lds, s, p, d, n_particles, lds, \
                         flags);                                                                                         \
    else                                                                                                                 \
      hipLaunchKernelGGL((k_likelihood<DN, IND, false>), dim3(grid), dim3(PFT_LIK_THREADS), lds, s, p, d, n_particles, lds, \
                         flags);                                                                                         \
  } while (0)
  if (debug_nn && leaf_indirect)
    PFT_LIK_LAUNCH(true, true);
  else if (debug_nn)
    PFT_LIK_LAUNCH(true, false);
  else if (leaf_indirect)
    PFT_LIK_LAUNCH(false, true);
  else
    PFT_LIK_LAUNCH(false, false);
#undef PFT_LIK_LAUNCH
}
```

pcl_tracking_amd/csrc/pft_octree.hip:

```cpp
#include "pft_device_utils.h"

#ifdef PFT_DIAG
#define STAMP(k) do { if (threadIdx.x == 0) d.hdr->ticks[k] = wall_clock64(); } while (0)
#define TICK_NOW() wall_clock64()
#else
#define STAMP(k) do { } while (0)
#define TICK_NOW() 0ull
#endif

#include "pft_octree_box.h"

#define PFT_REPLAY_HEAD 1024u
__device__ __forceinline__ void box_replay(BuildSh& S, const float4* __restrict__ pts, uint32_t n, double res, unsigned long long* hdr_ticks) {
  const uint32_t tid = threadIdx.x, nt = blockDim.x;
  const uint32_t head = n < PFT_REPLAY_HEAD ? n : PFT_REPLAY_HEAD;
  float lmn[3] = {FLT_MAX, FLT_MAX, FLT_MAX}, lmx[3] = {-FLT_MAX, -FLT_MAX, -FLT_MAX};
  const uint32_t wt = tid - WAVE, ws = nt - WAVE;
  auto local_aabb = [&]() {
    for (uint32_t i0 = PFT_REPLAY_HEAD + wt; i0 < n; i0 += 8u * ws) {
      float4 q[8];
#pragma unroll
      for (uint32_t k = 0; k < 8u; k++) q[k] = pts[min(i0 + k * ws, n - 1u)];
#pragma unroll
      for (uint32_t k = 0; k < 8u; k++) {
// ... 389 lines not shown
  st.each(n, [&](uint32_t, key_t& key, uint32_t& node) {
    uint32_t w = W[node];
    uint32_t c = key_child<key_t, B, Store::MORTON>(key, 0);
    uint32_t leaf = (w >> 8) + __popc(w & 0xffu & ((1u << c) - 1u));
    node = leaf;
    key = (key_t)atomicAdd(&W[leaf], 1u);
  });
  __syncthreads();
  {
    const uint32_t per = (n_leaves + nt - 1) / nt;
    const uint32_t a0 = leaf_start + min(n_leaves, tid * per), a1 = leaf_start + min(n_leaves, (tid + 1) * per);
    uint32_t cnt = 0;
    for (uint32_t nd = a0; nd < a1; nd++) cnt += W[nd];
    uint32_t total;
    uint32_t start = block_excl_scan<uint32_t>(cnt, S.u32s, &total);
    for (uint32_t nd = a0; nd < a1; nd++) {
      const uint32_t c = W[nd];
      W[nd] = start;
      start += c;
    }
  }
  if (tid == 0) {
    W[leaf_start + n_leaves] = n;
    S.variant = Store::CODE | (LDSW ? 8u : 0u) | (TMPLDS ? 16u : 0u);
  }
  __syncthreads();
  STAMP(4);
  uint32_t* TMP = TMPLDS ? lds_tmp : d.pt_tmp;
  st.each(n, [&](uint32_t i, key_t& key, uint32_t& node) { TMP[W[node] + (uint32_t)key] = i; });
  __syncthreads();
  STAMP(5);
  st.each(n, [&](uint32_t i, key_t&, uint32_t& node) {
    const uint32_t s = W[node], e = W[node + 1];
    uint32_t rank = 0;
    for (uint32_t k = s; k < e; k++) rank += TMP[k] < i ? 1u : 0u;
    d.leaf_order[s + rank] = i;
  });
  STAMP(6);
  const uint32_t n_words = leaf_start + n_leaves + 1;
  if (LDSW)
    for (uint32_t j = tid; j < n_words; j += nt) d.words[j] = W[j];
  *out_leaf_start = leaf_start;
  *out_n_leaves = n_leaves;
  return true;
}

template <class Store>
__device__ __forceinline__ void build_tree_any(const PftParams& prm, const PftDev& d, BuildSh& S, uint32_t n,
                                               uint32_t* lds_words, uint32_t cap, uint32_t* lds_tmp, uint32_t* ls,
                                               uint32_t* nl) {
  bool done = false;
  if (cap >= 64) {
    if (lds_tmp) done = build_tree<Store, true, true>(prm, d, S, n, lds_words, cap, lds_tmp, ls, nl);
    else done = build_tree<Store, true, false>(prm, d, S, n, lds_words, cap, lds_tmp, ls, nl);
  }
  __syncthreads();
  if (!done) build_tree<Store, false, false>(prm, d, S, n, lds_words, cap, lds_tmp, ls, nl);
}

template <int K>
__device__ __forceinline__ void build_hybrid(const PftParams& prm, const PftDev& d, BuildSh& S, uint32_t n, uint32_t* lds_words,
                             uint32_t cap, uint32_t* lds_tmp, uint32_t* ls, uint32_t* nl, int* path) {
  if (S.depth <= HybridStore<K>::B) {
    *path = 2;
    build_tree_any<HybridStore<K>>(prm, d, S, n, lds_words, cap, lds_tmp, ls, nl);
  } else {
    build_tree_any<GlobStore>(prm, d, S, n, lds_words, cap, lds_tmp, ls, nl);
  }
}

template <int K>
__device__ __forceinline__ void build_regs(const PftParams& prm, const PftDev& d, BuildSh& S, uint32_t n, uint32_t* lds_words,
                           uint32_t cap, uint32_t* lds_tmp, uint32_t* ls, uint32_t* nl, int* path) {
  if (S.depth <= RegStore<K>::B) {
    *path = 1;
    build_tree_any<RegStore<K>>(prm, d, S, n, lds_words, cap, lds_tmp, ls, nl);
  } else {
    build_tree_any<GlobStore>(prm, d, S, n, lds_words, cap, lds_tmp, ls, nl);
  }
}

template <bool GATED>
__global__ __launch_bounds__(PFT_BUILD_THREADS) void k_octree_build(PftParams prm, PftDev d, uint32_t lds_bytes,
                                                                    int copy_leaf_pts, int rescue) {
  extern __shared__ __attribute__((aligned(16))) unsigned char smem[];
  __shared__ BuildSh S;
  PftHeader* hdr = d.hdr;
  if (rescue && !(hdr->error & 8u)) return;
  const uint32_t tid = threadIdx.x;
  const float4 p_first = tid == 0 ? d.crop_pts[0] : make_float4(0, 0, 0, 0);
  const uint32_t n = hdr->n_crop;
  if (GATED && pft_unchanged(d.gate)) return;

  STAMP(0);
  if (tid == 0) {
    S.err = hdr->error & 4u;
    S.ngrow = 0;
    S.depth = 0;
    S.cur = 1;
    S.variant = 0;
    if (n > 0) box_init(S, p_first, prm.res);
  }
  __syncthreads();

  uint32_t* lds_u = reinterpret_cast<uint32_t*>(smem);
  const uint32_t lds_words_total = lds_bytes / 4u;
  uint32_t* lds_tmp = nullptr;
  uint32_t tmp_words = 0;
  if ((size_t)n * 5u / 2u + 64u <= lds_words_total) {
    lds_tmp = lds_u;
    tmp_words = (n + 3u) & ~3u;
  }
  uint32_t* lds_words = lds_u + tmp_words;
  const uint32_t cap = lds_words_total - tmp_words;

  uint32_t leaf_start = 0, n_leaves = 0;
  int path = 0;
  if (n > 0) {
    box_replay(S, d.crop_pts, n, prm.res, d.hdr->ticks);
    __syncthreads();
    STAMP(1);
  }
  if (n > 0 && !S.err) {
    if (n <= 4u * PFT_BUILD_THREADS) build_regs<4>(prm, d, S, n, lds_words, cap, lds_tmp, &leaf_start, &n_leaves, &path);
    else if (n <= 8u * PFT_BUILD_THREADS) build_regs<8>(prm, d, S, n, lds_words, cap, lds_tmp, &leaf_start, &n_leaves, &path);
    else if (n <= 14u * PFT_BUILD_THREADS) build_regs<14>(prm, d, S, n, lds_words, cap, lds_tmp, &leaf_start, &n_leaves, &path);
    else if (n <= 18u * PFT_BUILD_THREADS) build_hybrid<8>(prm, d, S, n, lds_words, cap, lds_tmp, &leaf_start, &n_leaves, &path);
    else build_tree_any<GlobStore>(prm, d, S, n, lds_words, cap, lds_tmp, &leaf_start, &n_leaves);
  }
  __syncthreads();
  STAMP(7);
  const int D = S.depth;
  const bool ok = n > 0 && !S.err && D > 0;
  if (copy_leaf_pts == 1 && ok) {
    __threadfence_block();
    for (uint32_t pos = tid; pos < n; pos += blockDim.x) d.leaf_pts[pos] = d.crop_pts[d.leaf_order[pos]];
  }

  const int use_table = (ok && D <= PFT_TABLE_MAX_DEPTH) ? 1 : 0;
  STAMP(8);
  if (tid == 0) {
    hdr->error = S.err;
    hdr->depth = D;
    hdr->use_table = use_table;
    hdr->n_grow = S.ngrow;
    hdr->build_path = path;
    const uint32_t lds_total = lds_bytes / 4u, var = S.variant;
    const bool tried = lds_total - ((size_t)n * 5u / 2u + 64u <= lds_total ? ((n + 3u) & ~3u) : 0u) >= 64u;
    hdr->build_variant = var | ((var && !(var & 8u) && tried) ? 32u : 0u) | ((ok && use_table && S.jump > 0) ? 64u : 0u) |
                         (rescue ? 128u : 0u) | ((uint32_t)copy_leaf_pts << 8);
    hdr->leaf_indirect = copy_leaf_pts == 2 ? 1 : 0;
    if (d.host_stat) d.host_stat[1] = (uint32_t)D;
    hdr->jump_level = (ok && use_table) ? S.jump : 0;
    hdr->n_leaves = ok ? n_leaves : 0;
    hdr->leaf_start = ok ? leaf_start : 0;
    hdr->n_words = ok ? leaf_start + n_leaves + 1 : 0;
  }
  if (tid == 64) {
    double maxabs = 0.0;
    for (int a = 0; a < 3; a++) maxabs = fmax(maxabs, fmax(fabs(S.mn[a]), fabs(S.mx[a])));
    const double eta = maxabs * 1.1920928955078125e-07;
    const double s_top = prm.res * (double)(1u << (D > 0 ? D - 1 : 0));
    const double E = 9.0 * eta + 40.0 * 5.9604644775390625e-08 * s_top;
    double mc = 2.0 * E / prm.res + 1.0e-3;
    hdr->margin_cells = (float)(mc < 0.25 ? mc : 1.0);
  }
  if (tid == 128) hdr->inv_res = (float)(1.0 / prm.res);
  if (tid == 320) pft_anc_window(hdr, d, D, ok && use_table && copy_leaf_pts == 0, S.mn, prm.res);
  if (tid >= 192 && tid < 195) {
    const int a = (int)tid - 192;
    hdr->ominf[a] = (float)S.mn[a];
    hdr->omin[a] = n > 0 ? S.mn[a] : 0.0;
    hdr->omax[a] = n > 0 ? S.mx[a] : 0.0;
  }
  if (tid >= 256 && tid < 256 + PFT_MAX_DEPTH + 3 && (int)tid - 256 <= D + 1) hdr->lvl_start[tid - 256] = S.lvl[tid - 256];
}

__device__ __forceinline__ void anc_fill(const PftDev& d, uint32_t gid, uint32_t stride) {
  const PftHeader* hdr = d.hdr;
  const int L = hdr->anc_level;
  if (L <= 0) return;
  const uint32_t bx = hdr->anc_bits[0], by = hdr->anc_bits[1], n = 1u << (bx + by + hdr->anc_bits[2]);
  const uint32_t x0 = hdr->anc_lo[0], y0 = hdr->anc_lo[1], z0 = hdr->anc_lo[2];
  const int J = hdr->jump_level <= L ? hdr->jump_level : 0;
  const uint32_t lvlJ = J > 0 ? hdr->lvl_start[J] : 0u;
  for (uint32_t c = gid; c < n; c += stride) {
    const uint32_t x = x0 + (c & ((1u << bx) - 1u)), y = y0 + ((c >> bx) & ((1u << by) - 1u)), z = z0 + (c >> (bx + by));
    uint32_t node = 0;
    int lvl = 0;
    if (J > 0) {
      const int sh = L - J;
      const uint32_t e = d.jump[(x >> sh) | ((y >> sh) << J) | ((z >> sh) << (2 * J))];
      node = e ? lvlJ + e - 1u : 0u;
      lvl = e ? J : 0;
    }
    for (; lvl < L; lvl++) {
      const int sh = L - lvl - 1;
      const uint32_t ch = (((x >> sh) & 1u) << 2) | (((y >> sh) & 1u) << 1) | ((z >> sh) & 1u);
      const uint32_t wv = d.words[node];
      if (!((wv >> ch) & 1u)) break;
      node = (wv >> 8) + __popc(wv & 0xffu & ((1u << ch) - 1u));
    }
    d.anc[c] = ((uint32_t)lvl << 27) | node;
  }
  if (gid == 0) d.hdr->anc_epoch = hdr->build_epoch;
}

template <bool GATED>
__global__ __launch_bounds__(256) void k_leaf_gather(PftDev d) {
  if (GATED && pft_unchanged(d.gate)) return;
  const PftHeader* hdr = d.hdr;
  const uint32_t pos = blockIdx.x * 256u + threadIdx.x;
  if (hdr->error || hdr->depth <= 0) return;
  if (pos < hdr->n_crop) d.leaf_pts[pos] = d.crop_pts[d.leaf_order[pos]];
  anc_fill(d, pos, gridDim.x * 256u);
}

#ifndef PFT_OCTREE_GATED_TU
extern template __global__ void k_octree_build<true>(PftParams, PftDev, uint32_t, int, int);
extern template __global__ void k_leaf_gather<true>(PftDev);

static void pftk_octree_set_attr() {
  static bool attr_set[PFT_MAX_DEVICES];
  const uint32_t lds = ((uint32_t)pftk_max_lds_bytes() - 10240u) & ~15u;
  const int dev = pftk_cur_device();
  if (!attr_set[dev])
    attr_set[dev] = hipFuncSetAttribute(reinterpret_cast<const void*>(&k_octree_build<false>),
                                        hipFuncAttributeMaxDynamicSharedMemorySize, (int)lds) == hipSuccess &&
                    hipFuncSetAttribute(reinterpret_cast<const void*>(&k_octree_build<true>),
                                        hipFuncAttributeMaxDynamicSharedMemorySize, (int)lds) == hipSuccess;
}

void pftk_octree(hipStream_t s, const PftParams& p, const PftDev& d, uint32_t expected_points, bool indirect) {
  const uint32_t lds = ((uint32_t)pftk_max_lds_bytes() - 10240u) & ~15u;
  pftk_octree_set_attr();
  const int mode = indirect ? 2 : (expected_points <= 5000u ? 1 : 0);
  const dim3 gg((d.N + 255u) / 256u ? (d.N + 255u) / 256u : 1u);
  if (d.gate) {
    hipLaunchKernelGGL(k_octree_build<true>, dim3(1), dim3(PFT_BUILD_THREADS), lds, s, p, d, lds, mode, 0);
    if (mode == 0) hipLaunchKernelGGL(k_leaf_gather<true>, gg, dim3(256), 0, s, d);
  } else {
    hipLaunchKernelGGL(k_octree_build<false>, dim3(1), dim3(PFT_BUILD_THREADS), lds, s, p, d, lds, mode, 0);
    if (mode == 0) hipLaunchKernelGGL(k_leaf_gather<false>, gg, dim3(256), 0, s, d);
  }
}

void pftk_octree_rescue(hipStream_t s, const PftParams& p, const PftDev& d) {
  pftk_octree_set_attr();
  const uint32_t lds = ((uint32_t)pftk_max_lds_bytes() - 10240u) & ~15u;
  if (d.gate)
    hipLaunchKernelGGL(k_octree_build<true>, dim3(1), dim3(PFT_BUILD_THREADS), lds, s, p, d, lds, 1, 1);
  else
    hipLaunchKernelGGL(k_octree_build<false>, dim3(1), dim3(PFT_BUILD_THREADS), lds, s, p, d, lds, 1, 1);
}
#endif
```

pcl_tracking_amd/csrc/pft_octree_gated.hip:

```cpp
#define PFT_OCTREE_GATED_TU
#include "pft_octree.hip"

template __global__ void k_octree_build<true>(PftParams, PftDev, uint32_t, int, int);
template __global__ void k_leaf_gather<true>(PftDev);
```

pcl_tracking_amd/csrc/pft_octree_sorted.hip:

```cpp
#include "pft_device_utils.h"

#define SO_TILE 1024
#define SO_BINS 256

struct ReplaySh {
  double mn[3], mx[3];
  int depth, ngrow;
  uint32_t cur, err;
  uint32_t u32s[40];
};

__device__ void so_box_grow(ReplaySh& S, PftHeader* hdr, float4 p, uint32_t idx, double res) {
  const double epsd = (double)FLT_EPSILON;
  for (;;) {
    bool lx = p.x < S.mn[0], ly = p.y < S.mn[1], lz = p.z < S.mn[2];
    bool ux = p.x >= S.mx[0], uy = p.y >= S.mx[1], uz = p.z >= S.mx[2];
    if (!(lx || ly || lz || ux || uy || uz)) break;
    int g = S.ngrow;
    if (g >= PFT_MAX_GROW || S.depth >= PFT_MAX_DEPTH) {
      S.err |= 2u;
      break;
    }
    double side = (double)(1u << S.depth) * res;
    hdr->grow_idx[g] = idx;
// ... 71 lines not shown
      unsigned mv = mk > 2u ? mk : 2u;
      double l2 = log((double)mv) / log(2.0);
      unsigned dep = (unsigned)ceil(l2 - (double)FLT_EPSILON);
      if (dep > 32u) dep = 32u;
      double side = (double)(1u << dep) * res - epsd;
      for (int a = 0; a < 3; a++) {
        double over = (side - (hi[a] - lo[a])) / 2.0;
        S.mn[a] = lo[a] - over;
        S.mx[a] = hi[a] + over;
        hdr->grow_min[0][a] = S.mn[a];
      }
      S.depth = (int)dep;
    }
  }
  __syncthreads();
  if (n > 1) {
    const uint32_t ntile = (n + SO_TILE - 1) / SO_TILE;
    for (;;) {
      const uint32_t cur = S.cur;
      if (cur >= n) break;
      const double mn[3] = {S.mn[0], S.mn[1], S.mn[2]};
      const double mx[3] = {S.mx[0], S.mx[1], S.mx[2]};
      uint32_t ft = 0xffffffffu;
      for (uint32_t t = cur / SO_TILE + tid; t < ntile; t += nt) {
        const float* b = tile_box + (size_t)t * 6;
        if (so_violates(b[0], b[1], b[2], mn, mx) || so_violates(b[3], b[4], b[5], mn, mx)) {
          ft = t;
          break;
        }
      }
      ft = block_reduce<uint32_t>(ft, S.u32s, OpMinU(), 0xffffffffu);
      if (ft == 0xffffffffu) break;
      uint32_t first = 0xffffffffu;
      {
        const uint32_t i = ft * SO_TILE + tid;
        if (i >= cur && i < n) {
          const float4 p = pts[i];
          if (so_violates(p.x, p.y, p.z, mn, mx)) first = i;
        }
      }
      first = block_reduce<uint32_t>(first, S.u32s + 20, OpMinU(), 0xffffffffu);
      if (tid == 0) {
        if (first == 0xffffffffu) {
          S.cur = (ft + 1) * SO_TILE;
        } else {
          so_box_grow(S, hdr, pts[first], first, res);
          S.cur = first + 1;
        }
      }
      __syncthreads();
      if (S.err) break;
    }
  }
  __syncthreads();
  const int D = S.depth;
  const bool ok = n > 0 && !S.err && D > 0;
  const int use_table = (ok && D <= PFT_TABLE_MAX_DEPTH) ? 1 : 0;
  const int J = (D >= 4 && D <= PFT_TABLE_MAX_DEPTH) ? (D - 1 < PFT_JUMP_MAX_LEVEL ? D - 1 : PFT_JUMP_MAX_LEVEL) : 0;
  if (J > 0) {
    uint32_t* jz = reinterpret_cast<uint32_t*>(d.jump);
    for (uint32_t j = tid; j < (1u << (3 * J - 1)); j += nt) jz[j] = 0u;
  }
  if (tid == 0) {
    hdr->error = S.err;
    hdr->depth = D;
    hdr->use_table = use_table;
    hdr->n_grow = S.ngrow;
    hdr->build_path = 2;
    hdr->leaf_indirect = 0;
    hdr->jump_level = (ok && use_table) ? J : 0;
    double maxabs = 0.0;
    for (int a = 0; a < 3; a++) maxabs = fmax(maxabs, fmax(fabs(S.mn[a]), fabs(S.mx[a])));
    const double eta = maxabs * 1.1920928955078125e-07;
    const double s_top = res * (double)(1u << (D > 0 ? D - 1 : 0));
    const double E = 9.0 * eta + 40.0 * 5.9604644775390625e-08 * s_top;
    double mc = 2.0 * E / res + 1.0e-3;
    hdr->margin_cells = (float)(mc < 0.25 ? mc : 1.0);
    for (int a = 0; a < 3; a++) {
      hdr->ominf[a] = (float)S.mn[a];
      hdr->omin[a] = n > 0 ? S.mn[a] : 0.0;
      hdr->omax[a] = n > 0 ? S.mx[a] : 0.0;
    }
    hdr->inv_res = (float)(1.0 / res);
    pft_anc_window(hdr, d, D, false, S.mn, res);
    if (!ok) {
      hdr->n_words = 0;
      hdr->n_leaves = 0;
      hdr->leaf_start = 0;
    }
  }
}

__global__ void k_so_keys(PftParams prm, PftDev d, SortBufs sb, uint32_t n_pad) {
  if (pft_unchanged(d.gate)) return;
  const uint32_t i = blockIdx.x * blockDim.x + threadIdx.x;
  if (i >= n_pad) return;
  const PftHeader* hdr = d.hdr;
  const uint32_t n = hdr->n_crop;
  const int D = hdr->depth, ngrow = hdr->n_grow;
  if (i >= n || hdr->error || D <= 0) return;
  const double res = prm.res, inv_res = 1.0 / prm.res;
  const float4 p = d.crop_pts[i];
  int e = 0;
  while (e < ngrow && hdr->grow_idx[e] <= i) e++;
  const double tq[3] = {(double)p.x - hdr->grow_min[e][0], (double)p.y - hdr->grow_min[e][1],
                        (double)p.z - hdr->grow_min[e][2]};
  uint32_t kk[3];
#pragma unroll
  for (int a = 0; a < 3; a++) {
    double q0 = tq[a] * inv_res;
    const double fr = q0 - floor(q0);
    if (fr < 1.0e-6 || fr > 1.0 - 1.0e-6) q0 = tq[a] / res;
    kk[a] = (uint32_t)q0;
  }
  for (int s = e; s < ngrow; s++) {
    const uint32_t sh = hdr->grow_shift[s], od = hdr->grow_old_depth[s];
    if (sh & 1u) kk[0] += 1u << od;
    if (sh & 2u) kk[1] += 1u << od;
    if (sh & 4u) kk[2] += 1u << od;
  }
  if (d.pt_key) {
    d.pt_key[3 * (size_t)i + 0] = kk[0];
    d.pt_key[3 * (size_t)i + 1] = kk[1];
    d.pt_key[3 * (size_t)i + 2] = kk[2];
  }
  unsigned long long code = 0;
  for (int b = D - 1; b >= 0; b--)
    code = (code << 3) | (unsigned long long)((((kk[0] >> b) & 1u) << 2) | (((kk[1] >> b) & 1u) << 1) | ((kk[2] >> b) & 1u));
  sb.keys[0][i] = code;
  sb.vals[0][i] = i;
}

__global__ __launch_bounds__(64) void k_rs_hist(const unsigned long long* __restrict__ keys, uint32_t n_pad, int shift,
                                                uint32_t* __restrict__ hist, uint32_t ntiles, const PftHeader* hdr,
                                                int pass, const uint32_t* gate) {
  if (pft_unchanged(gate)) return;
  if (pass * 8 >= 3 * hdr->depth && pass > 0) return;
  __shared__ uint32_t h[SO_BINS];
  const uint32_t t = blockIdx.x, lane = threadIdx.x;
  n_pad = hdr->error ? 0u : hdr->n_crop;
  for (int b = lane; b < SO_BINS; b += 64) h[b] = 0;
  __syncthreads();
  const uint32_t base = t * SO_TILE;
#pragma unroll 4
  for (int c = 0; c < SO_TILE / 64; c++) {
    const uint32_t i = base + c * 64 + lane;
    if (i < n_pad) atomicAdd(&h[(uint32_t)(keys[i] >> shift) & 0xffu], 1u);
  }
  __syncthreads();
  for (int b = lane; b < SO_BINS; b += 64) hist[(size_t)b * ntiles + t] = h[b];
}

__global__ __launch_bounds__(1024) void k_rs_scan(uint32_t* __restrict__ hist, uint32_t ntiles, const PftHeader* hdr,
                                                  int pass, const uint32_t* gate) {
  if (pft_unchanged(gate)) return;
  if (pass * 8 >= 3 * hdr->depth && pass > 0) return;
  __shared__ uint32_t scr[20];
  const uint32_t b = blockIdx.x, tid = threadIdx.x, nt = blockDim.x;
  uint32_t* row = hist + (size_t)b * ntiles;
  uint32_t carry = 0;
  for (uint32_t t0 = 0; t0 < ntiles; t0 += nt) {
    const uint32_t t = t0 + tid;
    const uint32_t v = t < ntiles ? row[t] : 0u;
    uint32_t tot;
    const uint32_t ex = block_excl_scan<uint32_t>(v, scr, &tot);
    if (t < ntiles) row[t] = carry + ex;
    carry += tot;
// ... 242 lines not shown
```

pcl_tracking_amd/tracker.py:

```python
import ctypes as C
from dataclasses import dataclass

import numpy as np

from . import _lib
from ._lib import Config, PftError

SUM_ORDERS = {"tree": _lib.PFT_SUM_TREE, "pcl": _lib.PFT_SUM_PCL}
from .scene import PARTICLE_DTYPE, POINT_DTYPE


def _ptr(a):
    return None if a is None else a.ctypes.data_as(C.c_void_p)


LIK_LAYOUTS = ("u16_leaf_starts", "u32_words", "branch_only", "hybrid")
LIK_DESCENTS = ("fast", "table_generic", "no_table")


def decode_likelihood_layout(out4):
    w = int(out4[0])
    return dict(valid=bool(w & 1), layout=LIK_LAYOUTS[(w >> 1) & 3], descent=LIK_DESCENTS[min((w >> 3) & 3, 2)],
                indirect=bool(w & 32), leaf_indirect=bool(w & 64), jump_dropped=bool(w & 128), J=(w >> 8) & 15,
                n_lds_words=int(out4[1]), lds_bytes=int(out4[2]), margin_cells=float(np.uint32(out4[3]).view(np.float32)))
# ... 659 lines not shown
        self._check(self._L.pft_eval_weights(self._h, _ptr(p), P, _ptr(raw), _ptr(nn_idx), _ptr(nn_d2)))
        bbox = np.zeros(6, np.float32)
        self._check(self._L.pft_debug_get_bbox(self._h, _ptr(bbox)))
        n = C.c_size_t()
        self._check(self._L.pft_debug_get_crop(self._h, None, 0, C.byref(n)))
        crop = np.zeros(n.value, np.int32)
        if n.value:
            self._check(self._L.pft_debug_get_crop(self._h, _ptr(crop), n.value, C.byref(n)))
        depth, nl, nn = C.c_int32(), C.c_uint32(), C.c_uint32()
        mn, mx = np.zeros(3), np.zeros(3)
        self._check(self._L.pft_debug_get_octree(self._h, C.byref(depth), _ptr(mn), _ptr(mx), C.byref(nl), C.byref(nn)))
        keys = np.zeros((n.value, 3), np.uint32)
        if n.value:
            self._check(self._L.pft_debug_get_point_keys(self._h, _ptr(keys), n.value))
        q, s = C.c_uint64(), C.c_uint64()
        self._check(self._L.pft_debug_get_scan_stats(self._h, C.byref(q), C.byref(s)))
        lay = np.zeros(4, np.uint32)
        self._check(self._L.pft_debug_get_likelihood_layout(self._h, _ptr(lay)))
        return dict(raw=raw, nn_idx=nn_idx, nn_d2=nn_d2, bbox=bbox, crop_idx=crop, octree_depth=depth.value,
                    octree_min=mn, octree_max=mx, n_leaves=nl.value, n_words=nn.value, point_keys=keys,
                    scan_queries=q.value, scan_points=s.value, lik_layout=decode_likelihood_layout(lay))

    def debugChangeState(self, which=0):
        self._ensure()
        gate, counter, n_calls = C.c_uint32(), C.c_uint32(), C.c_uint32()
        depth = C.c_int32()
        box = np.zeros(6, np.float64)
        ring = np.zeros((_lib.PFT_CD_RING, 5), np.uint32)
        self._check(self._L.pft_debug_change_state(self._h, which, C.byref(gate), C.byref(counter), _ptr(box),
                                                   C.byref(depth), _ptr(ring), C.byref(n_calls)))
        k = min(n_calls.value, _lib.PFT_CD_RING)
        return dict(gate=gate.value, counter=counter.value, box=box, depth=depth.value, ring=ring[:k].copy(),
                    n_calls=n_calls.value)

    def debugChangeDetect(self, cloud, min_points, resolution, reset):
        self._ensure()
        cloud = np.ascontiguousarray(cloud, POINT_DTYPE)
        out = np.zeros(max(len(cloud), 1), np.uint32)
        n = C.c_size_t()
        self._check(self._L.pft_debug_change_detect(self._h, _ptr(cloud), len(cloud), int(min_points), float(resolution),
                                                    int(bool(reset)), _ptr(out), len(out), C.byref(n)))
        return out[:n.value].copy()

    def debugSetLimits(self, max_words=0, sorted_npass=0):
        self._ensure()
        self._check(self._L.pft_debug_set_limits(self._h, int(max_words), int(sorted_npass)))

    def debugGetTree(self):
        self._ensure()
        info = np.zeros(_lib.PFT_TREE_INFO_WORDS, np.uint32)
        self._check(self._L.pft_debug_get_tree(self._h, _ptr(info), None, 0, None, 0, None, 0, None, 0, None, 0))
        n, n_words, n_jump = int(info[0]), int(info[4]), int(info[19])
        words = np.zeros(n_words, np.uint32)
        order = np.zeros(n, np.uint32)
        leaf_pts = np.zeros((n, 4), np.uint32)
        crop_pts = np.zeros((n, 4), np.uint32)
        jump = np.zeros(n_jump, np.uint16)
        self._check(self._L.pft_debug_get_tree(self._h, _ptr(info), _ptr(words), n_words, _ptr(order), n, _ptr(leaf_pts), n,
                                               _ptr(crop_pts), n, _ptr(jump), n_jump))
        names = ("n_crop", "error", "depth", "use_table", "n_words", "n_leaves", "leaf_start", "n_grow", "build_path",
                 "leaf_indirect", "jump_level", "margin_cells_bits", "inv_res_bits")
        out = {k: int(info[i]) for i, k in enumerate(names)}
        depth = out["depth"]
        out.update(ominf_bits=info[13:16].copy(), build_epoch=int(info[16]), build_variant=int(info[17]),
                   build_lds_bytes=int(info[18]), lvl_start=info[20:20 + depth + 2].copy() if depth > 0 else info[20:20].copy(),
                   words=words, leaf_order=order, leaf_pts=leaf_pts, crop_pts=crop_pts, jump=jump)
        return out

    def debugStateSave(self):
        self._check(self._L.pft_debug_state_save(self._h))

    def debugStateRestore(self):
        self._check(self._L.pft_debug_state_restore(self._h))

    def debugInjectError(self, bits):
        self._ensure()
        self._check(self._L.pft_debug_inject_error(self._h, int(bits)))

    def debugHostStat(self):
        self._ensure()
        out = np.zeros(4, np.uint32)
        self._check(self._L.pft_debug_get_host_stat(self._h, _ptr(out)))
        return out

    def debugNormalize(self, w):
        self._ensure()
        w = np.array(w, np.float32, copy=True)
        fr = C.c_double()
        self._check(self._L.pft_debug_normalize(self._h, _ptr(w), len(w), C.byref(fr)))
        return w, fr.value

    def debugAlias(self, w):
        self._ensure()
        w = np.ascontiguousarray(w, np.float32)
        a = np.zeros(len(w), np.int32)
        q = np.zeros(len(w), np.float64)
        self._check(self._L.pft_debug_alias(self._h, _ptr(w), len(w), _ptr(a), _ptr(q)))
        return a, q

    def debugWeightedMean(self, p):
        self._ensure()
        p = np.ascontiguousarray(p, PARTICLE_DTYPE)
        out = np.zeros(1, PARTICLE_DTYPE)
        self._check(self._L.pft_debug_weighted_mean(self._h, _ptr(p), len(p), _ptr(out)))
        return out[0]

    def debugInitParticles(self, rep, id_offset, n_local):
        self._ensure()
        rep = np.ascontiguousarray(rep, PARTICLE_DTYPE).reshape(1)
        out = np.zeros(n_local, PARTICLE_DTYPE)
        self._check(self._L.pft_debug_init_particles(self._h, _ptr(rep), id_offset, n_local, _ptr(out)))
        return out

    def debugResample(self, old, a, q, rep, epoch, id_offset=0, n_local=None):
        self._ensure()
        old = np.ascontiguousarray(old, PARTICLE_DTYPE)
        a = np.ascontiguousarray(a, np.int32)
        q = np.ascontiguousarray(q, np.float64)
        rep = np.ascontiguousarray(rep, PARTICLE_DTYPE).reshape(1)
        n_local = len(old) if n_local is None else n_local
        out = np.zeros(n_local, PARTICLE_DTYPE)
        self._check(self._L.pft_debug_resample(self._h, _ptr(old), len(old), _ptr(a), _ptr(q), _ptr(rep), epoch,
                                               id_offset, n_local, _ptr(out)))
        return out

    def debugResamplePrefix(self, old, rep, epoch, id_offset=0, n_local=None, instance=1, want_mats=False):
        self._ensure()
        old = np.ascontiguousarray(old, PARTICLE_DTYPE)
        rep = np.ascontiguousarray(rep, PARTICLE_DTYPE).reshape(1)
        n_local = len(old) if n_local is None else n_local
        out = np.zeros(n_local, PARTICLE_DTYPE)
        m = np.zeros((n_local, 12), np.float32) if want_mats else None
        self._check(self._L.pft_debug_resample_prefix(self._h, _ptr(old), len(old), _ptr(rep), epoch, id_offset, n_local,
                                                      int(instance), _ptr(out), _ptr(m) if want_mats else None))
        return (out, m.reshape(n_local, 3, 4)) if want_mats else out

    def debugPoseToMatrix(self, p):
        self._ensure()
        p = np.ascontiguousarray(p, PARTICLE_DTYPE)
        m = np.zeros((len(p), 12), np.float32)
        self._check(self._L.pft_debug_pose_to_matrix(self._h, _ptr(p), len(p), _ptr(m)))
        return m.reshape(len(p), 3, 4)

    def profileEnable(self, on=True):
        self._ensure()
        self._check(self._L.pft_profile_enable(self._h, 1 if on else 0))

    def profileReset(self):
        self._check(self._L.pft_profile_reset(self._h))

    def profileGet(self):
        out = {}
        for k in range(_lib.K_COUNT):
            ms, n = C.c_double(), C.c_uint64()
            self._check(self._L.pft_profile_get(self._h, k, C.byref(ms), C.byref(n)))
            out[self._L.pft_kernel_name(k).decode()] = (ms.value, n.value)
        return out


class KLDAdaptiveParticleFilterOMPTracker(ParticleFilterTracker):

    def __init__(self, *a, **kw):
        super().__init__(*a, **kw)
        self._cfg.kld_adaptive = 1

    def setMaximumParticleNum(self, n):
# ... 73 lines not shown
```

Before: 836.0 billion.

## Choose ancestor-table depth adaptively and specialize likelihood kernel on it

The ancestor lookup table can now be built one level above the leaves (anc_up=1) instead of always two levels up, whenever the bbox window fits within the capacity bits. The choice uses a device-written host status word plus a confirmation streak. The likelihood kernel is templated on ANC_UP, so descents start deeper and skip more octree traversal steps, and the table path is compiled out when unused. The cost is a larger table fill, extra kernel instances, and a cached graph that must be rebuilt whenever the chosen level sequence changes.

New measurement: 847.2 billion (median of 6 runs). 1.01x the previous value.

```diff
diff --git a/include/pft.h b/include/pft.h
--- a/include/pft.h
+++ b/include/pft.h
@@ -249,6 +249,7 @@
 int pft_debug_get_hard_steps(pft_tracker* t, uint64_t out5[5]);
 int pft_debug_get_likelihood_layout(pft_tracker* t, uint32_t out4[4]);
 int pft_debug_get_ancestor_table(pft_tracker* t, uint32_t info10[10], uint32_t* table, size_t cap);
+int pft_debug_get_ancestor_level(pft_tracker* t, uint32_t out5[5]);
 int pft_debug_aabb_support_subset(const pft_point_xyzrgba* pts, size_t n, uint32_t* keep, size_t* n_keep);
 #ifdef PFT_DIAG
 void pft_debug_set_ablate(pft_tracker* t, int mask);
diff --git a/pcl_tracking_amd/_lib.py b/pcl_tracking_amd/_lib.py
--- a/pcl_tracking_amd/_lib.py
+++ b/pcl_tracking_amd/_lib.py
@@ -203,6 +203,7 @@
     ("pft_debug_get_descent_stats", C.c_int, [_vp, _vp]),
     ("pft_debug_get_likelihood_layout", C.c_int, [_vp, _vp]),
     ("pft_debug_get_ancestor_table", C.c_int, [_vp, _vp, _vp, _sz]),
+    ("pft_debug_get_ancestor_level", C.c_int, [_vp, _vp]),
     ("pft_debug_get_hard_steps", C.c_int, [_vp, _vp]),
     ("pft_debug_aabb_support_subset", C.c_int, [_vp, C.c_size_t, _vp, _vp]),
     ("pft_debug_likelihood_occupancy", C.c_int, []),
diff --git a/pcl_tracking_amd/csrc/pft_api.hip b/pcl_tracking_amd/csrc/pft_api.hip
--- a/pcl_tracking_amd/csrc/pft_api.hip
+++ b/pcl_tracking_amd/csrc/pft_api.hip
@@ -178,6 +178,9 @@
   bool use_graph = false;
   hipGraphExec_t graph_exec = nullptr;
   uint32_t graph_frames = 0, graph_rebuilds = 0;
+  int anc_up_last = -1, lik_up_last = -1, graph_lik_up = -1;
+  uint32_t anc_up_changes = 0;
+  uint32_t anc_fit_streak = 0;
 
   bool prof = false;
   std::vector<EvPair> ev[PFT_K_COUNT];
@@ -565,6 +568,8 @@
   w.crop_two_pass = on("PFT_CROP_TWO_PASS");
   w.generic_descent = is1("PFT_GENERIC_DESCENT");
   w.ancestor_table = !on("PFT_ANCESTOR_TABLE") || is1("PFT_ANCESTOR_TABLE");
+  w.anc_up_force = -1;
+  if (const char* u = getenv("PFT_ANC_UP_FORCE")) w.anc_up_force = (u[0] >= '0' && u[0] <= '2' && !u[1]) ? u[0] - '0' : -1;
   w.exact_path = on("PFT_EXACT_SHELLS_ONLY") ? PftExactPath::shells : on("PFT_EXACT_PER_QUERY") ? PftExactPath::per_query : PftExactPath::sorted;
 #ifdef PFT_DIAG
   if (const char* a = getenv("PFT_ABLATE")) w.ablate = atoi(a);
@@ -1021,9 +1026,23 @@
 }
 __global__ void k_inject_error(PftHeader* hdr, uint32_t bits) { hdr->error |= bits; }
 
+#define PFT_ANC_UP_CONFIRM 8u
+static int pick_anc_up(pft_tracker* t, bool own_population, bool gather) {
+  if (!t->d_anc || !t->sw.ancestor_table || t->leaf_indirect || !gather) return 0;
+  if (t->sw.anc_up_force >= 0) return t->sw.anc_up_force;
+  const volatile uint32_t* hs = t->h_stat;
+  const uint32_t w = hs ? hs[5] : 0u;
+  if (!(w & 0x80000000u)) return 2;
+  if (own_population) {
+    t->anc_fit_streak = (w & 0xffu) <= PFT_ANC_CAP_BITS ? t->anc_fit_streak + 1u : 0u;
+    if (t->anc_fit_streak >= PFT_ANC_UP_CONFIRM) return 1;
+  }
+  return ((w >> 8) & 0xffu) <= PFT_ANC_CAP_BITS ? 2 : 0;
+}
+
 static void stage_crop_octree_likelihood(pft_tracker* t, const PftDev& d, uint32_t np, bool debug_nn,
                                          bool bbox_from_partials, bool keep_point_keys = false,
-                                         bool likelihood = true) {
+                                         bool likelihood = true, bool own_population = true) {
   {
     ProfScope ps(t, PFT_K_CROP);
     if (++t->crop_epoch == 0) t->crop_epoch = 1;
@@ -1111,6 +1130,7 @@
     pftk_likelihood_exact(t->stream, t->prm, dq, np, debug_nn, t->num_cus, t->sw.exact_path);
     return;
   }
+  int anc_up = 0;
   {
     ProfScope ps(t, PFT_K_OCTREE);
     PftDev db = d;
@@ -1132,14 +1152,17 @@
       t->leaf_indirect = false;
     } else {
       t->leaf_indirect = t->sw.leaf_indirect >= 0 ? t->sw.leaf_indirect == 1 : (unsigned long long)np * t->prm.M <= 8000000ull;
-      pftk_octree(t->stream, t->prm, db, last_n, t->leaf_indirect);
-    }
+      anc_up = pick_anc_up(t, own_population, last_n > PFT_GATHER_MIN);
+      pftk_octree(t->stream, t->prm, db, last_n, t->leaf_indirect, anc_up);
+    }
+    if (t->anc_up_last >= 0 && anc_up != t->anc_up_last) t->anc_up_changes++;
+    t->anc_up_last = anc_up;
   }
   if (!likelihood) return;
   {
     ProfScope ps(t, PFT_K_LIKELIHOOD);
     const int flags = (t->sw.generic_descent ? 0 : 1) | (t->sw.ancestor_table ? 2 : 0) | (t->sw.ablate << 8);
-    pftk_likelihood(t->stream, t->prm, d, np, debug_nn, t->num_cus, t->leaf_indirect, flags);
+    t->lik_up_last = pftk_likelihood(t->stream, t->prm, d, np, debug_nn, t->num_cus, t->leaf_indirect, flags, anc_up);
   }
 }
 
@@ -1172,11 +1195,14 @@
   }
   t->gate_on = t->cd_ever;
   sync_dev(t);
+  int lik_sig = 0;
   auto run_iterations = [&]() {
+    lik_sig = 0;
     for (int it = 0; it < t->cfg.iteration_num; it++) {
       stage_resample_aabb(t, false);
       const uint32_t np = t->prm.kld ? t->Pcap : t->prm.P_local;
       stage_crop_octree_likelihood(t, t->dev, np, false, true);
+      lik_sig = ((lik_sig << 2) | (t->lik_up_last + 1)) & 0xffffff;
       if (t->inject_error & 16u) {
         hipLaunchKernelGGL(k_inject_error, dim3(1), dim3(1), 0, t->stream, t->d_hdr, 16u);
         t->inject_error &= ~16u;
@@ -1206,6 +1232,11 @@
     }
     if (ge == hipSuccess && g) {
       bool ready = false;
+      if (t->graph_exec && t->graph_lik_up != lik_sig) {
+        hipGraphExecDestroy(t->graph_exec);
+        t->graph_exec = nullptr;
+      }
+      t->graph_lik_up = lik_sig;
       if (t->graph_exec) {
         hipGraphNode_t bad = nullptr;
         hipGraphExecUpdateResult res;
@@ -1542,7 +1573,7 @@
   HIPCHK(t, hipMemsetAsync(t->d_hdr->dbg_hard, 0, sizeof(t->d_hdr->dbg_hard) + sizeof(t->d_hdr->lik_layout), t->stream));
   pftk_pose_to_matrix(t->stream, t->d_dbg_part, (uint32_t)P, t->d_mats);
   stage_aabb(t, d, (uint32_t)P, false);
-  stage_crop_octree_likelihood(t, d, (uint32_t)P, want_nn, true, true);
+  stage_crop_octree_likelihood(t, d, (uint32_t)P, want_nn, true, true, true, false);
   pftk_finalize_raw(t->stream, t->prm, d, (uint32_t)P, t->d_dbg_f, nullptr);
   if (raw_w) HIPCHK(t, hipMemcpyAsync(raw_w, t->d_dbg_f, P * sizeof(float), hipMemcpyDeviceToHost, t->stream));
   if (nn_idx) HIPCHK(t, hipMemcpyAsync(nn_idx, t->d_nn_idx, pairs * sizeof(int32_t), hipMemcpyDeviceToHost, t->stream));
@@ -1706,6 +1737,17 @@
   int r = read_hdr(t, &h);
   if (r != PFT_OK) return r;
   memcpy(out4, h.lik_layout, sizeof(h.lik_layout));
+  return PFT_OK;
+}
+
+extern "C" int pft_debug_get_ancestor_level(pft_tracker* t, uint32_t out5[5]) {
+  if (!t || !out5 || !t->h_stat) return PFT_ERR_INVALID_ARG;
+  HIPCHK(t, hipStreamSynchronize(t->stream));
+  out5[0] = ((volatile uint32_t*)t->h_stat)[5];
+  out5[1] = (uint32_t)t->anc_up_last;
+  out5[2] = (uint32_t)t->lik_up_last;
+  out5[3] = t->anc_up_changes;
+  out5[4] = t->graph_rebuilds;
   return PFT_OK;
 }
 
diff --git a/pcl_tracking_amd/csrc/pft_device_utils.h b/pcl_tracking_amd/csrc/pft_device_utils.h
--- a/pcl_tracking_amd/csrc/pft_device_utils.h
+++ b/pcl_tracking_amd/csrc/pft_device_utils.h
@@ -216,28 +216,32 @@
 
 #include "pft_alias.h"
 
-__device__ inline void pft_anc_window(PftHeader* hdr, const PftDev& d, int D, bool on, const double mn[3], double res) {
-  const int L = D - PFT_ANC_UP;
-  on = on && d.anc != nullptr && L >= 1;
+__device__ inline void pft_anc_window(PftHeader* hdr, const PftDev& d, int D, bool on, bool fill, const double mn[3],
+                                      double res, int anc_up) {
+  const int L2 = D - 2;
+  on = on && d.anc != nullptr && L2 >= 0;
   const float inv = (float)(1.0 / res);
   uint32_t lo[3] = {0u, 0u, 0u}, bits[3] = {0u, 0u, 0u};
   for (int a = 0; a < 3 && on; a++) {
     const float om = (float)mn[a];
     const float f0 = fmaxf(floorf((hdr->bbox[2 * a] - om) * inv), 0.0f);
     const float f1 = fmaxf(floorf((hdr->bbox[2 * a + 1] - om) * inv), 0.0f);
-    const uint32_t top = (1u << L) - 1u;
-    const uint32_t c0 = min(f0 < 2147483648.0f ? (uint32_t)f0 >> PFT_ANC_UP : top, top);
-    const uint32_t c1 = min(f1 < 2147483648.0f ? (uint32_t)f1 >> PFT_ANC_UP : top, top);
+    const uint32_t top = (1u << L2) - 1u;
+    const uint32_t c0 = min(f0 < 2147483648.0f ? (uint32_t)f0 >> 2 : top, top);
+    const uint32_t c1 = min(f1 < 2147483648.0f ? (uint32_t)f1 >> 2 : top, top);
     on = c1 >= c0;
     const uint32_t n = c1 - c0 + 1u;
     bits[a] = n > 1u ? 32u - (uint32_t)__clz((int)(n - 1u)) : 0u;
-    lo[a] = min(c0, (1u << L) - (1u << bits[a]));
-  }
-  on = on && bits[0] + bits[1] + bits[2] <= PFT_ANC_CAP_BITS;
-  hdr->anc_level = on ? L : 0;
+    lo[a] = min(c0, (1u << L2) - (1u << bits[a]));
+  }
+  const uint32_t tb2 = bits[0] + bits[1] + bits[2], tb1 = tb2 + 3u;
+  if (d.host_stat) d.host_stat[5] = 0x80000000u | (on ? tb1 : 0xffu) | ((on && L2 >= 1 ? tb2 : 0xffu) << 8);
+  const bool deeper = anc_up == 1;
+  on = on && fill && (deeper ? tb1 <= PFT_ANC_CAP_BITS : (anc_up == 2 && L2 >= 1 && tb2 <= PFT_ANC_CAP_BITS));
+  hdr->anc_level = on ? D - anc_up : 0;
   for (int a = 0; a < 3; a++) {
-    hdr->anc_lo[a] = on ? lo[a] : 0u;
-    hdr->anc_bits[a] = on ? bits[a] : 0u;
+    hdr->anc_lo[a] = on ? (deeper ? 2u * lo[a] : lo[a]) : 0u;
+    hdr->anc_bits[a] = on ? (deeper ? bits[a] + 1u : bits[a]) : 0u;
   }
   hdr->build_epoch = hdr->build_epoch + 1u;
 }
diff --git a/pcl_tracking_amd/csrc/pft_internal.h b/pcl_tracking_amd/csrc/pft_internal.h
--- a/pcl_tracking_amd/csrc/pft_internal.h
+++ b/pcl_tracking_amd/csrc/pft_internal.h
@@ -15,9 +15,6 @@
 #define PFT_ANC_CAP_BITS 18
 #endif
 #define PFT_ANC_CAP (1u << PFT_ANC_CAP_BITS)
-#ifndef PFT_ANC_UP
-#define PFT_ANC_UP 2
-#endif
 #define PFT_REF_CHUNK 256
 #ifndef PFT_BUILD_THREADS
 #define PFT_BUILD_THREADS 1024
@@ -35,6 +32,7 @@
 #define PFT_LIK_WGS_PER_CU 2
 #endif
 #define PFT_POP_THREADS 1024
+#define PFT_GATHER_MIN 5000u
 #define PFT_SORTED_BUILD_MIN 18000
 #define PFT_EG_CAP (1u << 21)
 #define PFT_EC_SLOTS (1u << 19)
@@ -258,6 +256,7 @@
   bool crop_two_pass;
   bool generic_descent;
   bool ancestor_table;
+  int anc_up_force;
   PftExactPath exact_path;
   int ablate;
   bool skip_octree;
@@ -327,7 +326,7 @@
                        const int32_t* table_a, const double* table_q, int32_t* bins_out);
 void pftk_crop(hipStream_t s, const PftParams& p, const PftDev& d, bool bbox_from_partials, uint32_t epoch,
                const pft_point_xyzrgba* raw, bool two_pass, const uint32_t* n_src = nullptr);
-void pftk_octree(hipStream_t s, const PftParams& p, const PftDev& d, uint32_t expected_points, bool indirect);
+void pftk_octree(hipStream_t s, const PftParams& p, const PftDev& d, uint32_t expected_points, bool indirect, int anc_up);
 void pftk_octree_rescue(hipStream_t s, const PftParams& p, const PftDev& d);
 struct SortBufs {
   unsigned long long* keys[2];
@@ -339,8 +338,8 @@
 };
 void pftk_octree_sorted(hipStream_t s, const PftParams& p, const PftDev& d, const SortBufs& sb, uint32_t n_pad,
                         int npass);
-void pftk_likelihood(hipStream_t s, const PftParams& p, const PftDev& d, uint32_t n_particles, bool debug_nn,
-                     int num_cus, bool leaf_indirect, int flags);
+int pftk_likelihood(hipStream_t s, const PftParams& p, const PftDev& d, uint32_t n_particles, bool debug_nn,
+                    int num_cus, bool leaf_indirect, int flags, int anc_up);
 void pftk_finalize_raw(hipStream_t s, const PftParams& p, const PftDev& d, uint32_t n_particles,
                        float* raw_out , pft_particle* shard );
 void pftk_population(hipStream_t s, const PftParams& p, const PftDev& d, uint32_t n, int from_partials,
diff --git a/pcl_tracking_amd/csrc/pft_likelihood.hip b/pcl_tracking_amd/csrc/pft_likelihood.hip
--- a/pcl_tracking_amd/csrc/pft_likelihood.hip
+++ b/pcl_tracking_amd/csrc/pft_likelihood.hip
@@ -53,7 +53,7 @@
   return (low | high) ? (int)c : -1;
 }
 
-template <bool USE_TAB, bool FAST, bool DEBUG_NN, int LEAF, bool INDIRECT, typename WordPtr>
+template <bool USE_TAB, bool FAST, bool DEBUG_NN, int LEAF, bool INDIRECT, int ANC_UP, typename WordPtr>
 __device__ __forceinline__ void likelihood_items(const PftParams& prm, const PftDev& d, const LikCtx& cx, WordPtr W,
                                                  uint32_t n_particles, int D, uint32_t n_crop,
                                                  const double omin[3], int abl) {
@@ -130,26 +130,35 @@
         }
         V = inside ? V : 31;
         int lim = min(D, D - 1 - V);
-        bool inw = false;
-        uint32_t ae = 0u;
-        if (!INDIRECT && LEAF == 1 && cx.anc) {
-          const uint32_t bx = cx.abits & 0xffu, by = (cx.abits >> 8) & 0xffu, bz = cx.abits >> 16;
-          const uint32_t ux = (kx >> PFT_ANC_UP) - (cx.alo & 1023u), uy = (ky >> PFT_ANC_UP) - ((cx.alo >> 10) & 1023u),
-                         uz = (kz >> PFT_ANC_UP) - (cx.alo >> 20);
-          inw = ((ux >> bx) | (uy >> by) | (uz >> bz)) == 0u;
-          ae = cx.anc[inw ? ux | (uy << bx) | (uz << (bx + by)) : 0u];
-        }
-        const int a = (int)(ae >> 27);
-        const bool hit = inw & (a <= lim);
-        node = hit ? (ae & 0x7ffffffu) : 0u;
-        lvl = hit ? a : 0;
-        lim = (hit & (a < D - PFT_ANC_UP)) ? a : lim;
-        if (cx.J > 0 && __builtin_amdgcn_ballot_w64(!hit)) {
+        if constexpr (ANC_UP > 0 && !INDIRECT && LEAF == 1) {
+          bool inw = false;
+          uint32_t ae = 0u;
+          if (cx.anc) {
+            const uint32_t bx = cx.abits & 0xffu, by = (cx.abits >> 8) & 0xffu, bz = cx.abits >> 16;
+            const uint32_t ux = (kx >> ANC_UP) - (cx.alo & 1023u), uy = (ky >> ANC_UP) - ((cx.alo >> 10) & 1023u),
+                           uz = (kz >> ANC_UP) - (cx.alo >> 20);
+            inw = ((ux >> bx) | (uy >> by) | (uz >> bz)) == 0u;
+            ae = cx.anc[inw ? ux | (uy << bx) | (uz << (bx + by)) : 0u];
+          }
+          const int a = (int)(ae >> 27);
+          const bool hit = inw & (a <= lim);
+          node = hit ? (ae & 0x7ffffffu) : 0u;
+          lvl = hit ? a : 0;
+          lim = (hit & (a < D - ANC_UP)) ? a : lim;
+          if (cx.J > 0 && __builtin_amdgcn_ballot_w64(!hit)) {
+            const int sh = D - cx.J;
+            const uint32_t e = cx.jump[(kx >> sh) | ((ky >> sh) << cx.J) | ((kz >> sh) << (2 * cx.J))];
+            const bool take = !hit & (cx.J <= lim) & (e != 0u);
+            node = take ? cx.lvlJ_start + e - 1u : node;
+            lvl = take ? cx.J : lvl;
+            if (DEBUG_NN) dbg_jump = take ? 1 : 0;
+          }
+        } else if (cx.J > 0) {
           const int sh = D - cx.J;
           const uint32_t e = cx.jump[(kx >> sh) | ((ky >> sh) << cx.J) | ((kz >> sh) << (2 * cx.J))];
-          const bool take = !hit & (cx.J <= lim) & (e != 0u);
-          node = take ? cx.lvlJ_start + e - 1u : node;
-          lvl = take ? cx.J : lvl;
+          const bool take = (cx.J <= lim) & (e != 0u);
+          node = take ? cx.lvlJ_start + e - 1u : 0u;
+          lvl = take ? cx.J : 0;
           if (DEBUG_NN) dbg_jump = take ? 1 : 0;
         }
         while (lvl < lim) {
@@ -363,9 +372,9 @@
   }
 }
 
-#define PFT_LIK_RUN(UT, FA, LF) likelihood_items<UT, FA, DEBUG_NN, LF, INDIRECT>(prm, d, cx, W, n_particles, D, n_crop, omin, abl)
-
-template <bool DEBUG_NN, bool INDIRECT, bool GATED>
+#define PFT_LIK_RUN(UT, FA, LF) likelihood_items<UT, FA, DEBUG_NN, LF, INDIRECT, ANC_UP>(prm, d, cx, W, n_particles, D, n_crop, omin, abl)
+
+template <bool DEBUG_NN, bool INDIRECT, bool GATED, int ANC_UP>
 __global__ __launch_bounds__(PFT_LIK_THREADS, DEBUG_NN ? 1 : (PFT_LIK_THREADS * PFT_LIK_WGS_PER_CU) / 256) void k_likelihood(PftParams prm, PftDev d, uint32_t n_particles,
                                                                 uint32_t lds_bytes, int flags) {
   const int allow_fast = flags & 1;
@@ -469,7 +478,8 @@
   cx.jump = ljump;
   cx.J = J;
   cx.lvlJ_start = J > 0 ? hdr->lvl_start[J] : 0u;
-  const bool anc_on = fast && (flags & 2) && d.anc && hdr->anc_level > 0 && hdr->anc_epoch == hdr->build_epoch;
+  const bool anc_on = ANC_UP > 0 && fast && (flags & 2) && d.anc && hdr->anc_level > 0 && D - hdr->anc_level == ANC_UP &&
+                      hdr->anc_epoch == hdr->build_epoch;
   cx.anc = anc_on ? d.anc : nullptr;
   static_assert(PFT_TABLE_MAX_DEPTH <= 10, "ancestor table window coordinates are packed in 10 bits");
   cx.alo = hdr->anc_lo[0] | (hdr->anc_lo[1] << 10) | (hdr->anc_lo[2] << 20);
@@ -522,47 +532,53 @@
 extern "C" int pft_debug_likelihood_occupancy(void) {
   int nb = -1;
   uint32_t lds = ((uint32_t)pftk_max_lds_bytes() / (uint32_t)PFT_LIK_WGS_PER_CU) & ~255u;
-  hipFuncSetAttribute(reinterpret_cast<const void*>(&k_likelihood<false, false, false>), hipFuncAttributeMaxDynamicSharedMemorySize, (int)lds);
-  if (hipOccupancyMaxActiveBlocksPerMultiprocessor(&nb, reinterpret_cast<const void*>(&k_likelihood<false, false, false>), PFT_LIK_THREADS, lds) != hipSuccess) return -1;
+  hipFuncSetAttribute(reinterpret_cast<const void*>(&k_likelihood<false, false, false, 2>), hipFuncAttributeMaxDynamicSharedMemorySize, (int)lds);
+  if (hipOccupancyMaxActiveBlocksPerMultiprocessor(&nb, reinterpret_cast<const void*>(&k_likelihood<false, false, false, 2>), PFT_LIK_THREADS, lds) != hipSuccess) return -1;
   return nb;
 }
 
-void pftk_likelihood(hipStream_t s, const PftParams& p, const PftDev& d, uint32_t n_particles, bool debug_nn,
-                     int num_cus, bool leaf_indirect, int flags) {
+int pftk_likelihood(hipStream_t s, const PftParams& p, const PftDev& d, uint32_t n_particles, bool debug_nn,
+                    int num_cus, bool leaf_indirect, int flags, int anc_up) {
   static bool attr_set[PFT_MAX_DEVICES];
   uint32_t lds = ((uint32_t)pftk_max_lds_bytes() / (uint32_t)PFT_LIK_WGS_PER_CU) & ~255u;
   const int dev = pftk_cur_device();
+#define PFT_LIK_FN(DN, IND, GA, UP) reinterpret_cast<const void*>(&k_likelihood<DN, IND, GA, UP>)
   if (!attr_set[dev]) {
-    const void* fns[8] = {
-        reinterpret_cast<const void*>(&k_likelihood<false, false, false>), reinterpret_cast<const void*>(&k_likelihood<true, false, false>),
-        reinterpret_cast<const void*>(&k_likelihood<false, true, false>), reinterpret_cast<const void*>(&k_likelihood<true, true, false>),
-        reinterpret_cast<const void*>(&k_likelihood<false, false, true>), reinterpret_cast<const void*>(&k_likelihood<true, false, true>),
-        reinterpret_cast<const void*>(&k_likelihood<false, true, true>), reinterpret_cast<const void*>(&k_likelihood<true, true, true>)};
+    const void* fns[12] = {PFT_LIK_FN(false, false, false, 0), PFT_LIK_FN(false, false, false, 1), PFT_LIK_FN(false, false, false, 2),
+                           PFT_LIK_FN(false, false, true, 0),  PFT_LIK_FN(false, false, true, 1),  PFT_LIK_FN(false, false, true, 2),
+                           PFT_LIK_FN(true, false, false, 2),  PFT_LIK_FN(true, false, true, 2),   PFT_LIK_FN(false, true, false, 0),
+                           PFT_LIK_FN(false, true, true, 0),   PFT_LIK_FN(true, true, false, 0),   PFT_LIK_FN(true, true, true, 0)};
     bool ok = true;
-    for (int k = 0; k < 8; k++) ok = hipFuncSetAttribute(fns[k], hipFuncAttributeMaxDynamicSharedMemorySize, (int)lds) == hipSuccess && ok;
+    for (int k = 0; k < 12; k++) ok = hipFuncSetAttribute(fns[k], hipFuncAttributeMaxDynamicSharedMemorySize, (int)lds) == hipSuccess && ok;
     attr_set[dev] = ok;
   }
+#undef PFT_LIK_FN
   uint32_t items = n_particles * p.nchunk;
   uint32_t grid = (uint32_t)PFT_LIK_WGS_PER_CU * (uint32_t)num_cus;
   uint32_t need = (items + (PFT_LIK_THREADS / 64) - 1) / (PFT_LIK_THREADS / 64);
   if (need == 0) need = 1;
   if (grid > need) grid = need;
-#define PFT_LIK_LAUNCH(DN, IND)                                                                                          \
-  do {                                                                                                                   \
-    if (d.gate)                                                                                                          \
-      hipLaunchKernelGGL((k_likelihood<DN, IND, true>), dim3(grid), dim3(PFT_LIK_THREADS), lds, s, p, d, n_particles, lds, \
-                         flags);                                                                                         \
-    else                                                                                                                 \
-      hipLaunchKernelGGL((k_likelihood<DN, IND, false>), dim3(grid), dim3(PFT_LIK_THREADS), lds, s, p, d, n_particles, lds, \
-                         flags);                                                                                         \
+#define PFT_LIK_LAUNCH(DN, IND, UP)                                                                                          \
+  do {                                                                                                                       \
+    if (d.gate)                                                                                                              \
+      hipLaunchKernelGGL((k_likelihood<DN, IND, true, UP>), dim3(grid), dim3(PFT_LIK_THREADS), lds, s, p, d, n_particles, lds, \
+                         flags);                                                                                             \
+    else                                                                                                                     \
+      hipLaunchKernelGGL((k_likelihood<DN, IND, false, UP>), dim3(grid), dim3(PFT_LIK_THREADS), lds, s, p, d, n_particles, lds, \
+                         flags);                                                                                             \
+    return UP;                                                                                                               \
   } while (0)
   if (debug_nn && leaf_indirect)
-    PFT_LIK_LAUNCH(true, true);
+    PFT_LIK_LAUNCH(true, true, 0);
   else if (debug_nn)
-    PFT_LIK_LAUNCH(true, false);
+    PFT_LIK_LAUNCH(true, false, 2);
   else if (leaf_indirect)
-    PFT_LIK_LAUNCH(false, true);
+    PFT_LIK_LAUNCH(false, true, 0);
+  else if (anc_up == 1)
+    PFT_LIK_LAUNCH(false, false, 1);
+  else if (anc_up == 2)
+    PFT_LIK_LAUNCH(false, false, 2);
   else
-    PFT_LIK_LAUNCH(false, false);
+    PFT_LIK_LAUNCH(false, false, 0);
 #undef PFT_LIK_LAUNCH
 }
diff --git a/pcl_tracking_amd/csrc/pft_octree.hip b/pcl_tracking_amd/csrc/pft_octree.hip
--- a/pcl_tracking_amd/csrc/pft_octree.hip
+++ b/pcl_tracking_amd/csrc/pft_octree.hip
@@ -495,7 +495,7 @@
 
 template <bool GATED>
 __global__ __launch_bounds__(PFT_BUILD_THREADS) void k_octree_build(PftParams prm, PftDev d, uint32_t lds_bytes,
-                                                                    int copy_leaf_pts, int rescue) {
+                                                                    int copy_leaf_pts, int rescue, int anc_up) {
   extern __shared__ __attribute__((aligned(16))) unsigned char smem[];
   __shared__ BuildSh S;
   PftHeader* hdr = d.hdr;
@@ -579,7 +579,7 @@
     hdr->margin_cells = (float)(mc < 0.25 ? mc : 1.0);
   }
   if (tid == 128) hdr->inv_res = (float)(1.0 / prm.res);
-  if (tid == 320) pft_anc_window(hdr, d, D, ok && use_table && copy_leaf_pts == 0, S.mn, prm.res);
+  if (tid == 320) pft_anc_window(hdr, d, D, ok && use_table, copy_leaf_pts == 0, S.mn, prm.res, anc_up);
   if (tid >= 192 && tid < 195) {
     const int a = (int)tid - 192;
     hdr->ominf[a] = (float)S.mn[a];
@@ -593,28 +593,49 @@
   const PftHeader* hdr = d.hdr;
   const int L = hdr->anc_level;
   if (L <= 0) return;
-  const uint32_t bx = hdr->anc_bits[0], by = hdr->anc_bits[1], n = 1u << (bx + by + hdr->anc_bits[2]);
-  const uint32_t x0 = hdr->anc_lo[0], y0 = hdr->anc_lo[1], z0 = hdr->anc_lo[2];
-  const int J = hdr->jump_level <= L ? hdr->jump_level : 0;
+  const bool deeper = hdr->depth - L == 1;
+  const int Lw = deeper ? L - 1 : L;
+  const uint32_t bx = hdr->anc_bits[0], by = hdr->anc_bits[1], bz = hdr->anc_bits[2];
+  const uint32_t wbx = deeper ? bx - 1u : bx, wby = deeper ? by - 1u : by, wbz = deeper ? bz - 1u : bz;
+  const uint32_t n = 1u << (wbx + wby + wbz);
+  const uint32_t x0 = hdr->anc_lo[0] >> (deeper ? 1 : 0), y0 = hdr->anc_lo[1] >> (deeper ? 1 : 0),
+                 z0 = hdr->anc_lo[2] >> (deeper ? 1 : 0);
+  const int J = hdr->jump_level <= Lw ? hdr->jump_level : 0;
   const uint32_t lvlJ = J > 0 ? hdr->lvl_start[J] : 0u;
   for (uint32_t c = gid; c < n; c += stride) {
-    const uint32_t x = x0 + (c & ((1u << bx) - 1u)), y = y0 + ((c >> bx) & ((1u << by) - 1u)), z = z0 + (c >> (bx + by));
+    const uint32_t ux = c & ((1u << wbx) - 1u), uy = (c >> wbx) & ((1u << wby) - 1u), uz = c >> (wbx + wby);
+    const uint32_t x = x0 + ux, y = y0 + uy, z = z0 + uz;
     uint32_t node = 0;
     int lvl = 0;
     if (J > 0) {
-      const int sh = L - J;
+      const int sh = Lw - J;
       const uint32_t e = d.jump[(x >> sh) | ((y >> sh) << J) | ((z >> sh) << (2 * J))];
       node = e ? lvlJ + e - 1u : 0u;
       lvl = e ? J : 0;
     }
-    for (; lvl < L; lvl++) {
-      const int sh = L - lvl - 1;
+    for (; lvl < Lw; lvl++) {
+      const int sh = Lw - lvl - 1;
       const uint32_t ch = (((x >> sh) & 1u) << 2) | (((y >> sh) & 1u) << 1) | ((z >> sh) & 1u);
       const uint32_t wv = d.words[node];
       if (!((wv >> ch) & 1u)) break;
       node = (wv >> 8) + __popc(wv & 0xffu & ((1u << ch) - 1u));
     }
-    d.anc[c] = ((uint32_t)lvl << 27) | node;
+    const uint32_t own = ((uint32_t)lvl << 27) | node;
+    if (!deeper) {
+      d.anc[c] = own;
+    } else {
+      const uint32_t wv = lvl == Lw ? d.words[node] : 0u;
+      const uint32_t mask = wv & 0xffu, base = wv >> 8;
+#pragma unroll
+      for (uint32_t yz = 0; yz < 4u; yz++) {
+        const uint32_t c0 = yz, c1 = 4u | yz;
+        uint2 e;
+        e.x = (mask >> c0) & 1u ? ((uint32_t)L << 27) | (base + __popc(mask & ((1u << c0) - 1u))) : own;
+        e.y = (mask >> c1) & 1u ? ((uint32_t)L << 27) | (base + __popc(mask & ((1u << c1) - 1u))) : own;
+        const uint32_t idx = (2u * ux) | ((2u * uy + (yz >> 1)) << bx) | ((2u * uz + (yz & 1u)) << (bx + by));
+        *reinterpret_cast<uint2*>(d.anc + idx) = e;
+      }
+    }
   }
   if (gid == 0) d.hdr->anc_epoch = hdr->build_epoch;
 }
@@ -630,7 +651,7 @@
 }
 
 #ifndef PFT_OCTREE_GATED_TU
-extern template __global__ void k_octree_build<true>(PftParams, PftDev, uint32_t, int, int);
+extern template __global__ void k_octree_build<true>(PftParams, PftDev, uint32_t, int, int, int);
 extern template __global__ void k_leaf_gather<true>(PftDev);
 
 static void pftk_octree_set_attr() {
@@ -644,16 +665,16 @@
                                         hipFuncAttributeMaxDynamicSharedMemorySize, (int)lds) == hipSuccess;
 }
 
-void pftk_octree(hipStream_t s, const PftParams& p, const PftDev& d, uint32_t expected_points, bool indirect) {
+void pftk_octree(hipStream_t s, const PftParams& p, const PftDev& d, uint32_t expected_points, bool indirect, int anc_up) {
   const uint32_t lds = ((uint32_t)pftk_max_lds_bytes() - 10240u) & ~15u;
   pftk_octree_set_attr();
-  const int mode = indirect ? 2 : (expected_points <= 5000u ? 1 : 0);
+  const int mode = indirect ? 2 : (expected_points <= PFT_GATHER_MIN ? 1 : 0);
   const dim3 gg((d.N + 255u) / 256u ? (d.N + 255u) / 256u : 1u);
   if (d.gate) {
-    hipLaunchKernelGGL(k_octree_build<true>, dim3(1), dim3(PFT_BUILD_THREADS), lds, s, p, d, lds, mode, 0);
+    hipLaunchKernelGGL(k_octree_build<true>, dim3(1), dim3(PFT_BUILD_THREADS), lds, s, p, d, lds, mode, 0, anc_up);
     if (mode == 0) hipLaunchKernelGGL(k_leaf_gather<true>, gg, dim3(256), 0, s, d);
   } else {
-    hipLaunchKernelGGL(k_octree_build<false>, dim3(1), dim3(PFT_BUILD_THREADS), lds, s, p, d, lds, mode, 0);
+    hipLaunchKernelGGL(k_octree_build<false>, dim3(1), dim3(PFT_BUILD_THREADS), lds, s, p, d, lds, mode, 0, anc_up);
     if (mode == 0) hipLaunchKernelGGL(k_leaf_gather<false>, gg, dim3(256), 0, s, d);
   }
 }
@@ -662,8 +683,8 @@
   pftk_octree_set_attr();
   const uint32_t lds = ((uint32_t)pftk_max_lds_bytes() - 10240u) & ~15u;
   if (d.gate)
-    hipLaunchKernelGGL(k_octree_build<true>, dim3(1), dim3(PFT_BUILD_THREADS), lds, s, p, d, lds, 1, 1);
+    hipLaunchKernelGGL(k_octree_build<true>, dim3(1), dim3(PFT_BUILD_THREADS), lds, s, p, d, lds, 1, 1, 0);
   else
-    hipLaunchKernelGGL(k_octree_build<false>, dim3(1), dim3(PFT_BUILD_THREADS), lds, s, p, d, lds, 1, 1);
+    hipLaunchKernelGGL(k_octree_build<false>, dim3(1), dim3(PFT_BUILD_THREADS), lds, s, p, d, lds, 1, 1, 0);
 }
 #endif
diff --git a/pcl_tracking_amd/csrc/pft_octree_gated.hip b/pcl_tracking_amd/csrc/pft_octree_gated.hip
--- a/pcl_tracking_amd/csrc/pft_octree_gated.hip
+++ b/pcl_tracking_amd/csrc/pft_octree_gated.hip
@@ -1,5 +1,5 @@
 #define PFT_OCTREE_GATED_TU
 #include "pft_octree.hip"
 
-template __global__ void k_octree_build<true>(PftParams, PftDev, uint32_t, int, int);
+template __global__ void k_octree_build<true>(PftParams, PftDev, uint32_t, int, int, int);
 template __global__ void k_leaf_gather<true>(PftDev);
diff --git a/pcl_tracking_amd/csrc/pft_octree_sorted.hip b/pcl_tracking_amd/csrc/pft_octree_sorted.hip
--- a/pcl_tracking_amd/csrc/pft_octree_sorted.hip
+++ b/pcl_tracking_amd/csrc/pft_octree_sorted.hip
@@ -177,7 +177,7 @@
       hdr->omax[a] = n > 0 ? S.mx[a] : 0.0;
     }
     hdr->inv_res = (float)(1.0 / res);
-    pft_anc_window(hdr, d, D, false, S.mn, res);
+    pft_anc_window(hdr, d, D, false, false, S.mn, res, 0);
     if (!ok) {
       hdr->n_words = 0;
       hdr->n_leaves = 0;
diff --git a/pcl_tracking_amd/tracker.py b/pcl_tracking_amd/tracker.py
--- a/pcl_tracking_amd/tracker.py
+++ b/pcl_tracking_amd/tracker.py
@@ -765,6 +765,16 @@
         out = np.zeros(4, np.uint32)
         self._check(self._L.pft_debug_get_host_stat(self._h, _ptr(out)))
         return out
+
+    def debugAncestorLevel(self):
+        self._ensure()
+        o = np.zeros(5, np.uint32)
+        self._check(self._L.pft_debug_get_ancestor_level(self._h, _ptr(o)))
+        st = int(o[0])
+        b1, b2 = st & 0xFF, (st >> 8) & 0xFF
+        valid = bool(st >> 31)
+        return dict(status=st, bits_d1=b1 if valid and b1 != 0xFF else None, bits_d2=b2 if valid and b2 != 0xFF else None,
+                    anc_up=int(np.int32(o[1])), instance=int(np.int32(o[2])), changes=int(o[3]), graph_builds=int(o[4]))
 
     def debugNormalize(self, w):
         self._ensure()
```
